# stcodeer/Frequency-wised_All-in-One_Image_Restoration_Model

Measured on AMD Instinct MI355X. Metric: training images/sec @128x128, higher is better.
Workload: dtype bf16; 1 GPU; BASELINE configs[1]: Uformer encoder+decoder (all_3_bands, L=3, freq MSA), denoise sigma=25, 128x128, phase-2 train step (fwd+bwd+Adam, DropPath on); per_gpu_batch=16, global_batch=16, parallelism=dp1, hip_graph=True

## Files before the change

frequency-wised_all-in-one_image_restoration_model_amd/csrc/fw_common.h:

```cpp
#pragma once
#include <hip/hip_runtime.h>
#include <stdint.h>
#include <mutex>

#define FW_DT_F32 0
#define FW_DT_BF16 1

typedef __attribute__((ext_vector_type(4))) float f32x4;
typedef __attribute__((ext_vector_type(8))) __bf16 bf16x8_t;
typedef unsigned short bf16raw;

#define FW_DEV static __device__ __forceinline__
#define FW_SPEC __device__ __forceinline__
#define FW_MEM __device__ __forceinline__

FW_DEV int lane_id() { return threadIdx.x & 63; }

FW_DEV float bf2f(bf16raw b) { return __uint_as_float(((unsigned)b) << 16); }
FW_DEV bf16raw f2bf(float f) {
    __bf16 h = (__bf16)f;
    return __builtin_bit_cast(bf16raw, h);
}
typedef __attribute__((ext_vector_type(2))) float fw_f32x2;
typedef __attribute__((ext_vector_type(2))) __bf16 fw_bf16x2;
// ... 139 lines not shown
}
template <> FW_SPEC void store_acc_T<bf16raw>(char* dst, int ldb, int row0, int col0, const f32x4& acc) {
    const int l = lane_id();
    uint2 v = make_uint2(pack_bf2(acc[0], acc[1]), pack_bf2(acc[2], acc[3]));
    *reinterpret_cast<uint2*>(dst + (col0 + (l & 15)) * ldb + (row0 + ((l >> 4) << 2)) * 2) = v;
}
template <typename T> FW_DEV void store_acc_N(char* dst, int ldb, int row0, int col0, const f32x4& acc) {
    const int l = lane_id();
    char* p = dst + (row0 + ((l >> 4) << 2)) * ldb + (col0 + (l & 15)) * TT<T>::SZ;
#pragma unroll
    for (int r = 0; r < 4; ++r) TT<T>::st(reinterpret_cast<T*>(p + r * ldb), acc[r]);
}

template <typename T, int MT, int NT>
FW_DEV void mma_tiles(f32x4 (&acc)[MT][NT], const char* A, int lda, int a_row0, const char* B, int ldb,
                      int b_row0, int KC) {
    for (int c = 0; c < KC; ++c) {
        uint4 af[MT], bfr[NT];
#pragma unroll
        for (int m = 0; m < MT; ++m) af[m] = frag_kc(A, lda, a_row0 + 16 * m, c);
#pragma unroll
        for (int n = 0; n < NT; ++n) bfr[n] = frag_kc(B, ldb, b_row0 + 16 * n, c);
#pragma unroll
        for (int m = 0; m < MT; ++m)
#pragma unroll
            for (int n = 0; n < NT; ++n) mma_chunk<T>(acc[m][n], af[m], bfr[n]);
    }
}

template <int MT, int NT> FW_DEV void zero_acc(f32x4 (&acc)[MT][NT]) {
#pragma unroll
    for (int m = 0; m < MT; ++m)
#pragma unroll
        for (int n = 0; n < NT; ++n) acc[m][n] = f32x4{0.f, 0.f, 0.f, 0.f};
}

#define FW_MFMA_F32(acc, a, b) acc = __builtin_amdgcn_mfma_f32_16x16x4f32(a, b, acc, 0, 0, 0)

FW_DEV f32x4 frag_g(const float* P, int pitch, int row0, int c) {
    const int l = lane_id();
    return *reinterpret_cast<const f32x4*>(P + (size_t)(row0 + (l & 15)) * pitch + c * 16 + ((l >> 4) << 2));
}

template <bool REAL_IN, bool REAL_OUT, bool PANEL_FIRST> struct DftChunk {
    f32x4 ar[2], ai[2], pc[2], p1[2], p2[2];
    FW_MEM void load_panels(int t, const float* P, int pitch, int p0, int c, bool conj) {
        const size_t plane = (size_t)pitch * pitch;
        pc[t] = frag_g(P, pitch, p0 + 16 * t, c);
        if (!REAL_IN) p1[t] = frag_g(P + (conj ? 2 : 1) * plane, pitch, p0 + 16 * t, c);
        if (!REAL_OUT) p2[t] = frag_g(P + (conj ? 1 : 2) * plane, pitch, p0 + 16 * t, c);
    }
    FW_MEM void load_data(int t, const float* xr, const float* xi, int pitch, int d0, int c) {
        ar[t] = frag_g(xr, pitch, d0 + 16 * t, c);
        if (!REAL_IN) ai[t] = frag_g(xi, pitch, d0 + 16 * t, c);
    }
    FW_MEM void load(const float* xr, const float* xi, int dpitch, int d0, const float* P, int ppitch, int p0, int c, bool conj) {
#pragma unroll
        for (int t = 0; t < 2; ++t) {
            load_data(t, xr, xi, dpitch, d0, c);
            load_panels(t, P, ppitch, p0, c, conj);
        }
    }
    FW_MEM void mac(f32x4 (&accr)[2][2], f32x4 (&acci)[2][2]) const {
#pragma unroll
        for (int s = 0; s < 4; ++s)
#pragma unroll
            for (int mt = 0; mt < 2; ++mt)
#pragma unroll
                for (int nt = 0; nt < 2; ++nt) {
                    const int d = PANEL_FIRST ? nt : mt, p = PANEL_FIRST ? mt : nt;
#define FW_CHUNK_MAC(acc, x, pn) FW_MFMA_F32(acc, PANEL_FIRST ? pn[p][s] : x[d][s], PANEL_FIRST ? x[d][s] : pn[p][s])
                    FW_CHUNK_MAC(accr[mt][nt], ar, pc);
                    if (!REAL_OUT) FW_CHUNK_MAC(acci[mt][nt], ar, p2);
                    if (!REAL_IN) {
                        FW_CHUNK_MAC(accr[mt][nt], ai, p1);
                        if (!REAL_OUT) FW_CHUNK_MAC(acci[mt][nt], ai, pc);
                    }
#undef FW_CHUNK_MAC
                }
    }
    FW_MEM void mac(f32x4 (&acc)[2][2]) const { mac(acc, acc); }
};

#define FW_CHECK_ARG(cond)                                                                   \
    do {                                                                                     \
        if (!(cond)) return -__LINE__;                                                       \
    } while (0)
#define FW_LAUNCH_RET()                                                                      \
    do {                                                                                     \
        hipError_t e__ = hipGetLastError();                                                  \
        return e__ == hipSuccess ? 0 : (int)e__;                                             \
    } while (0)

#define FW_SET_LDS_ONCE(kern, bytes)                                                         \
    do {                                                                                     \
        static std::once_flag once__;                                                        \
        std::call_once(once__, [&] {                                                         \
            (void)hipFuncSetAttribute(reinterpret_cast<const void*>(kern), hipFuncAttributeMaxDynamicSharedMemorySize, (int)(bytes)); \
        });                                                                                  \
    } while (0)

static inline int fw_cdiv(long a, long b) { return (int)((a + b - 1) / b); }
```

frequency-wised_all-in-one_image_restoration_model_amd/csrc/fw_elem.hip:

```cpp
#include "fw_common.h"
#include <stdlib.h>

namespace {

constexpr int TPB = 256;
FW_DEV long gtid() { return (long)blockIdx.x * TPB + threadIdx.x; }
FW_DEV long gstride() { return (long)gridDim.x * TPB; }
static inline int grid_for(long n, int cap = 8192) { long g = (n + TPB - 1) / TPB; return (int)(g < 1 ? 1 : (g > cap ? cap : g)); }

template <typename T> FW_DEV void ldvec(const T* p, float* f) {
    unpack16<T>(*reinterpret_cast<const uint4*>(p), f);
}
template <typename T> FW_DEV void stvec(T* p, const float* f) { *reinterpret_cast<uint4*>(p) = pack16<T>(f); }
template <typename T> FW_DEV void ldvec4(const T* p, float* f);
template <> FW_SPEC void ldvec4<float>(const float* p, float* f) { unpack16<float>(*reinterpret_cast<const uint4*>(p), f); }
template <> FW_SPEC void ldvec4<bf16raw>(const bf16raw* p, float* f) {
    const uint2 v = *reinterpret_cast<const uint2*>(p);
    f[0] = __uint_as_float(v.x << 16); f[1] = __uint_as_float(v.x & 0xffff0000u);
    f[2] = __uint_as_float(v.y << 16); f[3] = __uint_as_float(v.y & 0xffff0000u);
}
template <typename T> FW_DEV void stvec4(T* p, const float* f);
template <> FW_SPEC void stvec4<float>(float* p, const float* f) { *reinterpret_cast<uint4*>(p) = pack16<float>(f); }
template <> FW_SPEC void stvec4<bf16raw>(bf16raw* p, const float* f) {
    *reinterpret_cast<uint2*>(p) = make_uint2(pack_bf2(f[0], f[1]), pack_bf2(f[2], f[3]));
// ... 712 lines not shown
        else *reinterpret_cast<uint2*>(d) = make_uint2(pack_bf2(v[0], v[1]), pack_bf2(v[2], v[3]));
    }
}
template <typename T>
__global__ void col2im4_kernel(const T* __restrict__ dcol, float* __restrict__ dx, long lddx, const float* __restrict__ dres, long ldr,
                               int B, int H, int W, int C) {
    const int Ho = H / 2, Wo = W / 2, c4n = C >> 2;
    const long total = (long)B * H * W * c4n;
    for (long i = gtid(); i < total; i += gstride()) {
        const int c = (int)(i % c4n) * 4; const long tok = i / c4n;
        const int x = (int)(tok % W); const int y = (int)((tok / W) % H); const long b = tok / ((long)W * H);
        f32x4 acc = f32x4{0.f, 0.f, 0.f, 0.f};
        if (dres) acc = *reinterpret_cast<const f32x4*>(dres + tok * ldr + c);
        for (int ky = (y + 1) & 1; ky < 4; ky += 2) {
            const int oy = (y + 1 - ky) / 2;
            if (y + 1 - ky < 0 || oy >= Ho) continue;
            for (int kx = (x + 1) & 1; kx < 4; kx += 2) {
                const int ox = (x + 1 - kx) / 2;
                if (x + 1 - kx < 0 || ox >= Wo) continue;
                const T* s = dcol + (((b * Ho + oy) * Wo + ox) * 16 + ky * 4 + kx) * (long)C + c;
                for (int e = 0; e < 4; ++e) acc[e] += TT<T>::ld(s + e);
            }
        }
        *reinterpret_cast<f32x4*>(dx + tok * lddx + c) = acc;
    }
}

template <typename T>
__global__ __launch_bounds__(1024) void im2col4_run_kernel(const float* __restrict__ x, long ldx, T* __restrict__ col, int B, int H, int W, int C,
                                                           int ipb) {
    const int Ho = H / 2, Wo = W / 2, c4n = C >> 2, Q = 4 * c4n;
    const int il = threadIdx.x / Q, q = threadIdx.x - il * Q;
    if (il >= ipb) return;
    const int kx = q / c4n, c = (q - kx * c4n) * 4;
    const unsigned ntok = (unsigned)B * Ho * Wo;
    for (unsigned t = blockIdx.x * ipb + il; t < ntok; t += gridDim.x * ipb) {
        const unsigned ox = t % Wo, t2 = t / Wo, oy = t2 % Ho, b = t2 / Ho;
        const int ix = 2 * (int)ox - 1 + kx, iy0 = 2 * (int)oy - 1;
        const bool okx = ix >= 0 && ix < W;
        const float* px = x + (((long)b * H) * W + min(max(ix, 0), W - 1)) * ldx + c;
        f32x4 v[4];
#pragma unroll
        for (int ky = 0; ky < 4; ++ky) v[ky] = *reinterpret_cast<const f32x4*>(px + (long)min(max(iy0 + ky, 0), H - 1) * W * ldx);
        T* d = col + ((long)t * 16 + kx) * C + c;
#pragma unroll
        for (int ky = 0; ky < 4; ++ky) {
            const bool ok = okx && iy0 + ky >= 0 && iy0 + ky < H;
            const f32x4 u = ok ? v[ky] : f32x4{0.f, 0.f, 0.f, 0.f};
            if (sizeof(T) == 4) *reinterpret_cast<f32x4*>(d + (long)ky * 4 * C) = u;
            else *reinterpret_cast<uint2*>(d + (long)ky * 4 * C) = make_uint2(pack_bf2(u[0], u[1]), pack_bf2(u[2], u[3]));
        }
    }
}
template <typename T>
__global__ __launch_bounds__(1024) void col2im4_run_kernel(const T* __restrict__ dcol, float* __restrict__ dx, long lddx, const float* __restrict__ dres,
                                                           long ldr, int B, int H, int W, int C, int ipb) {
    const int Ho = H / 2, Wo = W / 2, c4n = C >> 2;
    const int il = threadIdx.x / c4n, c = (threadIdx.x - il * c4n) * 4;
    if (il >= ipb) return;
    const unsigned ntok = (unsigned)B * H * W;
    for (unsigned tok = blockIdx.x * ipb + il; tok < ntok; tok += gridDim.x * ipb) {
        const unsigned xx = tok % W, t2 = tok / W, yy = t2 % H, b = t2 / H;
        const int x = (int)xx, y = (int)yy;
        const int ky0 = (y + 1) & 1, kx0 = (x + 1) & 1;
        float f[4][4];
        bool ok[4];
#pragma unroll
        for (int i = 0; i < 2; ++i)
#pragma unroll
            for (int j = 0; j < 2; ++j) {
                const int ky = ky0 + 2 * i, kx = kx0 + 2 * j;
                const int ny = y + 1 - ky, nx = x + 1 - kx;
                ok[i * 2 + j] = ny >= 0 && ny < 2 * Ho && nx >= 0 && nx < 2 * Wo;
                const int oy = min(max(ny, 0) >> 1, Ho - 1), ox = min(max(nx, 0) >> 1, Wo - 1);
                ldvec4<T>(dcol + ((((long)b * Ho + oy) * Wo + ox) * 16 + ky * 4 + kx) * (long)C + c, f[i * 2 + j]);
            }
        f32x4 acc = f32x4{0.f, 0.f, 0.f, 0.f};
        if (dres) acc = *reinterpret_cast<const f32x4*>(dres + (long)tok * ldr + c);
#pragma unroll
        for (int k = 0; k < 4; ++k)
#pragma unroll
            for (int e = 0; e < 4; ++e) acc[e] = ok[k] ? acc[e] + f[k][e] : acc[e];
        *reinterpret_cast<f32x4*>(dx + (long)tok * lddx + c) = acc;
    }
}

template <typename T>
__global__ void pixel_shuffle_kernel(const T* __restrict__ g, const float* __restrict__ bias, float* __restrict__ out, long ldo,
                                     int B, int H, int W, int Cout) {
    const int c4n = Cout >> 2;
    const long total = (long)B * H * W * 4 * c4n;
    for (long i = gtid(); i < total; i += gstride()) {
        const int c = (int)(i % c4n) * 4; long t = i / c4n;
        const int q = (int)(t % 4); t /= 4;
        const int x = (int)(t % W); const int y = (int)((t / W) % H); const long b = t / ((long)W * H);
        const T* s = g + t * 4L * Cout + q * Cout + c;
        float* d = out + ((b * 2 * H + 2 * y + (q >> 1)) * 2 * W + 2 * x + (q & 1)) * ldo + c;
        f32x4 v;
        for (int e = 0; e < 4; ++e) v[e] = TT<T>::ld(s + e) + bias[c + e];
        *reinterpret_cast<f32x4*>(d) = v;
    }
}
template <typename T>
__global__ void pixel_unshuffle_kernel(const float* __restrict__ dout, long ldo, T* __restrict__ dg, int B, int H, int W, int Cout) {
    const int c4n = Cout >> 2;
    const long total = (long)B * H * W * 4 * c4n;
    for (long i = gtid(); i < total; i += gstride()) {
        const int c = (int)(i % c4n) * 4; long t = i / c4n;
        const int q = (int)(t % 4); t /= 4;
        const int x = (int)(t % W); const int y = (int)((t / W) % H); const long b = t / ((long)W * H);
        const float* s = dout + ((b * 2 * H + 2 * y + (q >> 1)) * 2 * W + 2 * x + (q & 1)) * ldo + c;
        T* d = dg + t * 4L * Cout + q * Cout + c;
        for (int e = 0; e < 4; ++e) TT<T>::st(d + e, s[e]);
    }
}
__global__ void colsum_kernel(const float* __restrict__ x, long ldx, float* __restrict__ out, long rows, int cols, int rows_per_block) {
    const long r0 = (long)blockIdx.x * rows_per_block;
    for (int c = threadIdx.x; c < cols; c += TPB) {
        float s = 0.f;
        for (long r = r0; r < rows && r < r0 + rows_per_block; ++r) s += x[r * ldx + c];
        atomicAdd(out + c, s);
    }
}
__global__ __launch_bounds__(256) void colsum4_kernel(const float* __restrict__ x, long ldx, float* __restrict__ out, long rows, int cols, int rows_per_block) {
    __shared__ f32x4 red[TPB];
    const int nv = cols >> 2, rl = TPB / nv;
    const int v = threadIdx.x % nv, lane = threadIdx.x / nv;
    const long r0 = (long)blockIdx.x * rows_per_block;
    const long r1 = r0 + rows_per_block < rows ? r0 + rows_per_block : rows;
    f32x4 s = f32x4{0.f, 0.f, 0.f, 0.f};
    if (lane < rl) {
#pragma unroll 4
        for (long r = r0 + lane; r < r1; r += rl) s += *reinterpret_cast<const f32x4*>(x + r * ldx + 4 * v);
    }
    red[threadIdx.x] = s;
    __syncthreads();
    if (threadIdx.x < nv) {
        f32x4 t = red[threadIdx.x];
        for (int j = 1; j < rl; ++j) t += red[j * nv + threadIdx.x];
#pragma unroll
        for (int e = 0; e < 4; ++e) atomicAdd(out + 4 * threadIdx.x + e, t[e]);
    }
}
template <typename T>
__global__ void colsum_t_kernel(const T* __restrict__ x, long ldx, float* __restrict__ out, long rows, int cols, int rows_per_block) {
    const long r0 = (long)blockIdx.x * rows_per_block;
    for (int c = threadIdx.x; c < cols; c += TPB) {
        float s = 0.f;
        for (long r = r0; r < rows && r < r0 + rows_per_block; ++r) s += TT<T>::ld(x + r * ldx + c);
        atomicAdd(out + c, s);
    }
}

constexpr int EC_TY = 8, EC_TX = 32, EC_PH = EC_TY + 2, EC_PW = EC_TX + 2, EC_PLANE = EC_PH * EC_PW, EC_PN = 3 * EC_PLANE, EC_PIX = EC_TY * EC_TX;
constexpr int EC_PREG = (EC_PN + 255) / 256;
struct EcTiles {
    int tx, ty; long n;
    __device__ EcTiles(int B, int H, int W) : tx((W + EC_TX - 1) / EC_TX), ty((H + EC_TY - 1) / EC_TY) { n = (long)B * tx * ty; }
    __device__ void at(long t, long& b, int& y0, int& x0) const { x0 = (int)(t % tx) * EC_TX; y0 = (int)((t / tx) % ty) * EC_TY; b = t / ((long)tx * ty); }
};
FW_DEV void ec_patch_load(float (&r)[EC_PREG], const float* __restrict__ src, const EcTiles& T, long t, int H, int W) {
    long b; int y0, x0;
    T.at(t, b, y0, x0);
#pragma unroll
    for (int k = 0; k < EC_PREG; ++k) {
        int i = threadIdx.x + k * 256; i = i < EC_PN ? i : EC_PN - 1;
// ... 505 lines not shown
    FW_CHECK_ARG(dh2 && h1 && w && dh1 && dw && dbias && C % e == 0 && ld1 % e == 0 && ldg % e == 0 && ldo % e == 0 && W % SX == 0);
    FW_CHECK_ARG(ldg == ld1);
    FW_CHECK_ARG(B > 0 && H > 0 && W > 0 && C > 0 && ld1 >= C && ldo >= C);
    const long n = (long)B * H * (W / SX) * (C / 4);
    const int nvg = (C / 4 + WG_VL - 1) / WG_VL;
    const long nst = (long)B * H * (W / SX);
    constexpr int NSTRIP_MAX = 16;
    constexpr long wg_min_blocks = 384;
    int NSTRIP = NSTRIP_MAX;
    while (NSTRIP > 2 && ((nst + (long)NSTRIP * WG_SL - 1) / ((long)NSTRIP * WG_SL)) * nvg < wg_min_blocks) NSTRIP >>= 1;
    const long nsg = (nst + (long)NSTRIP * WG_SL - 1) / ((long)NSTRIP * WG_SL);
    const dim3 gridw((unsigned)(nsg * nvg));
    const bool tiled = dw_tiled(B, H, W, C);
    if (tiled && !g1 && (long)H * W * ldg < (1L << 31)) {
        constexpr long want = 1024;
        const long ncol = (long)((C + DT_CB - 1) / DT_CB) * ((W + DT_TX - 1) / DT_TX), nrow = (long)B * (H / DT_TY);
        long NT = ncol * nrow / want;
        NT = NT < 1 ? 1 : (NT > 32 ? 32 : NT);
        long nb = ncol * ((nrow + NT - 1) / NT);
        nb = (nb + 7) / 8 * 8;
        const size_t esz = dtype == FW_DT_BF16 ? 2 : 4;
        const size_t lds = (size_t)(DT_TY + 2) * ((DT_TX + 2) * DT_CB * esz + 128) + (9 * DT_CB + 40 * 256) * sizeof(float);
        if (dtype == FW_DT_BF16) {
            FW_SET_LDS_ONCE((dwconv_bwd_fused_kernel<bf16raw>), lds);
            hipLaunchKernelGGL((dwconv_bwd_fused_kernel<bf16raw>), dim3((unsigned)nb), dim3(256), lds, ST, (const bf16raw*)dh2, ldg, (const bf16raw*)h1, w,
                               (bf16raw*)dh1, ldo, dw, dbias, B, H, W, C, (int)NT);
        } else {
            FW_SET_LDS_ONCE((dwconv_bwd_fused_kernel<float>), lds);
            hipLaunchKernelGGL((dwconv_bwd_fused_kernel<float>), dim3((unsigned)nb), dim3(256), lds, ST, (const float*)dh2, ldg, (const float*)h1, w,
                               (float*)dh1, ldo, dw, dbias, B, H, W, C, (int)NT);
        }
        FW_LAUNCH_RET();
    }
    if (tiled) {
        const int rc = dtype == FW_DT_BF16
            ? dwconv_tile_launch<bf16raw, 1>((const bf16raw*)dh2, ldg, w, (const float*)nullptr, (const bf16raw*)h1, (bf16raw*)dh1, (bf16raw*)nullptr, ldo, B, H, W, C, ST)
            : dwconv_tile_launch<float, 1>((const float*)dh2, ldg, w, (const float*)nullptr, (const float*)h1, (float*)dh1, (float*)nullptr, ldo, B, H, W, C, ST);
        if (rc) return rc;
    }
    if (dtype == FW_DT_BF16) {
        if (!tiled) hipLaunchKernelGGL((dwconv_strip_kernel<bf16raw, 1>), dim3((grid_for(n) + 7) / 8 * 8), dim3(TPB), 0, ST, (const bf16raw*)dh2, ldg, w, (const float*)nullptr,
                           (const bf16raw*)h1, (bf16raw*)dh1, (bf16raw*)nullptr, ldo, B, H, W, C);
        if (g1) hipLaunchKernelGGL((dwconv_wgrad_kernel<bf16raw, false>), gridw, dim3(256), 0, ST, (const bf16raw*)dh2, ldg, (const bf16raw*)g1, ld1, dw, dbias, B, H, W, C, NSTRIP);
        else hipLaunchKernelGGL((dwconv_wgrad_kernel<bf16raw, true>), gridw, dim3(256), 0, ST, (const bf16raw*)dh2, ldg, (const bf16raw*)h1, ld1, dw, dbias, B, H, W, C, NSTRIP);
    } else {
        if (!tiled) hipLaunchKernelGGL((dwconv_strip_kernel<float, 1>), dim3((grid_for(n) + 7) / 8 * 8), dim3(TPB), 0, ST, (const float*)dh2, ldg, w, (const float*)nullptr,
                           (const float*)h1, (float*)dh1, (float*)nullptr, ldo, B, H, W, C);
        if (g1) hipLaunchKernelGGL((dwconv_wgrad_kernel<float, false>), gridw, dim3(256), 0, ST, (const float*)dh2, ldg, (const float*)g1, ld1, dw, dbias, B, H, W, C, NSTRIP);
        else hipLaunchKernelGGL((dwconv_wgrad_kernel<float, true>), gridw, dim3(256), 0, ST, (const float*)dh2, ldg, (const float*)h1, ld1, dw, dbias, B, H, W, C, NSTRIP);
    }
    FW_LAUNCH_RET();
}
extern "C" int fw_im2col4(int dtype, const float* x, long ldx, void* col, int B, int H, int W, int C, void* stream) {
    FW_CHECK_ARG(x && col && C % 4 == 0 && ldx % 4 == 0 && H % 2 == 0 && W % 2 == 0);
    const long n = (long)B * (H / 2) * (W / 2) * 16 * (C / 4);
    const long ntok = (long)B * (H / 2) * (W / 2);
    if (C >= 4 && C <= 1024 && ntok > 0 && ntok < (1L << 31) - (1L << 24) && ((uintptr_t)x & 15) == 0 &&
        ((uintptr_t)col & (dtype == FW_DT_BF16 ? 7 : 15)) == 0) {
        const int ipb = C >= 256 ? 1 : 256 / C;
        const dim3 g((unsigned)run_grid(ntok, ipb)), b((unsigned)((ipb * C + 63) / 64 * 64));
        if (dtype == FW_DT_BF16) hipLaunchKernelGGL((im2col4_run_kernel<bf16raw>), g, b, 0, ST, x, ldx, (bf16raw*)col, B, H, W, C, ipb);
        else hipLaunchKernelGGL((im2col4_run_kernel<float>), g, b, 0, ST, x, ldx, (float*)col, B, H, W, C, ipb);
        FW_LAUNCH_RET();
    }
    if (dtype == FW_DT_BF16) LAUNCH((im2col4_kernel<bf16raw>), n, x, ldx, (bf16raw*)col, B, H, W, C);
    LAUNCH((im2col4_kernel<float>), n, x, ldx, (float*)col, B, H, W, C);
}
extern "C" int fw_col2im4(int dtype, const void* dcol, float* dx, long lddx, const float* dres, long ldr, int B, int H, int W, int C,
                          void* stream) {
    FW_CHECK_ARG(dcol && dx && C % 4 == 0 && lddx % 4 == 0 && H % 2 == 0 && W % 2 == 0 && (!dres || ldr % 4 == 0));
    const long n = (long)B * H * W * (C / 4);
    const long ntok = (long)B * H * W;
    if (C >= 4 && C <= 4096 && ntok > 0 && ntok < (1L << 31) - (1L << 24) && (((uintptr_t)dx | (uintptr_t)dres) & 15) == 0 &&
        ((uintptr_t)dcol & (dtype == FW_DT_BF16 ? 7 : 15)) == 0) {
        const int c4n = C / 4, ipb = c4n >= 256 ? 1 : 256 / c4n;
        const dim3 g((unsigned)run_grid(ntok, ipb)), b((unsigned)((ipb * c4n + 63) / 64 * 64));
        if (dtype == FW_DT_BF16) hipLaunchKernelGGL((col2im4_run_kernel<bf16raw>), g, b, 0, ST, (const bf16raw*)dcol, dx, lddx, dres, ldr, B, H, W, C, ipb);
        else hipLaunchKernelGGL((col2im4_run_kernel<float>), g, b, 0, ST, (const float*)dcol, dx, lddx, dres, ldr, B, H, W, C, ipb);
        FW_LAUNCH_RET();
    }
    if (dtype == FW_DT_BF16) LAUNCH((col2im4_kernel<bf16raw>), n, (const bf16raw*)dcol, dx, lddx, dres, ldr, B, H, W, C);
    LAUNCH((col2im4_kernel<float>), n, (const float*)dcol, dx, lddx, dres, ldr, B, H, W, C);
}
extern "C" int fw_pixel_shuffle(int dtype, const void* g, const float* bias, float* out, long ldo, int B, int H, int W, int Cout,
                                void* stream) {
    FW_CHECK_ARG(g && bias && out && Cout % 4 == 0 && ldo % 4 == 0);
    const long n = (long)B * H * W * Cout;
    if (dtype == FW_DT_BF16) LAUNCH((pixel_shuffle_kernel<bf16raw>), n, (const bf16raw*)g, bias, out, ldo, B, H, W, Cout);
    LAUNCH((pixel_shuffle_kernel<float>), n, (const float*)g, bias, out, ldo, B, H, W, Cout);
}
extern "C" int fw_pixel_unshuffle(int dtype, const float* dout, long ldo, void* dg, int B, int H, int W, int Cout, void* stream) {
    FW_CHECK_ARG(dout && dg && Cout % 4 == 0 && ldo % 4 == 0);
    const long n = (long)B * H * W * Cout;
    if (dtype == FW_DT_BF16) LAUNCH((pixel_unshuffle_kernel<bf16raw>), n, dout, ldo, (bf16raw*)dg, B, H, W, Cout);
    LAUNCH((pixel_unshuffle_kernel<float>), n, dout, ldo, (float*)dg, B, H, W, Cout);
}
extern "C" int fw_colsum(int x_dtype, const void* x, long ldx, float* out, long rows, int cols, void* stream) {
    FW_CHECK_ARG(x && out && rows > 0 && cols > 0);
    int rpb = (int)((rows + 1023) / 1024);
    if (rpb < 32) rpb = 32;
    int grid = (int)((rows + rpb - 1) / rpb);
    if (x_dtype != 1 && cols % 4 == 0 && cols <= 512 && ldx % 4 == 0 && ((uintptr_t)x & 15) == 0 && ((uintptr_t)out & 3) == 0) {
        rpb = (int)((rows + 255) / 256);
        if (rpb < 32) rpb = 32;
        grid = (int)((rows + rpb - 1) / rpb);
        hipLaunchKernelGGL(colsum4_kernel, dim3(grid), dim3(TPB), 0, ST, (const float*)x, ldx, out, rows, cols, rpb);
        FW_LAUNCH_RET();
    }
    if (x_dtype == 1) hipLaunchKernelGGL((colsum_t_kernel<bf16raw>), dim3(grid), dim3(TPB), 0, ST, (const bf16raw*)x, ldx, out, rows, cols, rpb);
    else hipLaunchKernelGGL(colsum_kernel, dim3(grid), dim3(TPB), 0, ST, (const float*)x, ldx, out, rows, cols, rpb);
    FW_LAUNCH_RET();
}
#ifndef FW_EC_WGRAD_CAP
#define FW_EC_WGRAD_CAP 512
#endif
static inline int ec_grid(int B, int H, int W, int cap) {
    const long n = (long)B * ((H + EC_TY - 1) / EC_TY) * ((W + EC_TX - 1) / EC_TX);
    return (int)(n < cap ? n : cap);
}
static inline bool ec_al16(const void* p) { return ((uintptr_t)p & 15) == 0; }
constexpr int OP_PROD_BYTES = ((EC_PLANE + 15) / 16) * 16 * OP_PS * 4;
constexpr int OP_MAX_C = 896;
extern "C" int fw_inproj_fwd(const float* img, const float* w, const float* bias, float* out, long ldo, int B, int H, int W, int C,
                             float slope, void* stream) {
    FW_CHECK_ARG(img && w && bias && out && C % 4 == 0 && ldo % 4 == 0 && C > 0 && C <= 1024 && B > 0 && H > 0 && W > 0);
    FW_CHECK_ARG(ec_al16(out) && ec_al16(bias));
    hipLaunchKernelGGL(edge_conv3_rows_kernel<0>, dim3(ec_grid(B, H, W, 768)), dim3(TPB), 0, ST, img, w, bias, out, ldo, B, H, W, C, slope);
    FW_LAUNCH_RET();
}
extern "C" int fw_inproj_bwd(const float* img, const float* out, long ldo, const float* dy, long ldy, float* dw, float* db, int B,
                             int H, int W, int C, float slope, void* stream) {
    FW_CHECK_ARG(img && out && dy && dw && db && C > 0 && B > 0 && H > 0 && W > 0);
    const dim3 grid(ec_grid(B, H, W, FW_EC_WGRAD_CAP));
    const bool v4 = C % 4 == 0 && ldo % 4 == 0 && ldy % 4 == 0 && ec_al16(out) && ec_al16(dy);
    const int slice = v4 ? 1024 : 256;
    for (int c0 = 0; c0 < C; c0 += slice) {
        const int cs = C - c0 < slice ? C - c0 : slice;
        if (v4) hipLaunchKernelGGL((edge_conv3_wgrad_kernel<4, 0>), grid, dim3(TPB), 0, ST, img, dy + c0, ldy, out + c0, ldo, dw + (long)c0 * 27, db + c0, B, H, W, cs, slope);
        else hipLaunchKernelGGL((edge_conv3_wgrad_kernel<1, 0>), grid, dim3(TPB), 0, ST, img, dy + c0, ldy, out + c0, ldo, dw + (long)c0 * 27, db + c0, B, H, W, cs, slope);
    }
    FW_LAUNCH_RET();
}
extern "C" int fw_outproj_fwd(const float* fea, long ldf, const float* w, const float* bias, const float* img, float* out, int B,
                              int H, int W, int C, void* stream) {
    FW_CHECK_ARG(fea && w && bias && out && C % 4 == 0 && ldf % 4 == 0 && C > 0 && C <= OP_MAX_C && B > 0 && H > 0 && W > 0 && ec_al16(fea));
    const size_t lds = (size_t)((C + 15) / 16) * 2048 + OP_PROD_BYTES;
    FW_SET_LDS_ONCE(outproj_fwd_mfma_kernel, (OP_MAX_C / 16) * 2048 + OP_PROD_BYTES);
    hipLaunchKernelGGL(outproj_fwd_mfma_kernel, dim3(ec_grid(B, H, W, 512)), dim3(TPB), lds, ST, fea, ldf, w, bias, img, out, B, H, W, C);
    FW_LAUNCH_RET();
}
extern "C" int fw_outproj_bwd(const float* dout, const float* fea, long ldf, const float* w, float* dfea, long lddf, float* dw,
                              float* db, int B, int H, int W, int C, void* stream) {
    FW_CHECK_ARG(dout && fea && w && dfea && dw && db && C % 4 == 0 && ldf % 4 == 0 && lddf % 4 == 0 && C > 0 && C <= 1024 && B > 0 && H > 0 && W > 0);
    FW_CHECK_ARG(ec_al16(fea) && ec_al16(dfea));
    hipLaunchKernelGGL(edge_conv3_rows_kernel<1>, dim3(ec_grid(B, H, W, 768)), dim3(TPB), 0, ST, dout, w, (const float*)nullptr, dfea, lddf, B, H, W, C, 0.f);
    hipLaunchKernelGGL((edge_conv3_wgrad_kernel<4, 1>), dim3(ec_grid(B, H, W, FW_EC_WGRAD_CAP)), dim3(TPB), 0, ST, dout, fea, ldf, (const float*)nullptr, 0L, dw, db,
                       B, H, W, C, 0.f);
    FW_LAUNCH_RET();
}
extern "C" int fw_l1_loss(const float* a, const float* b, float* da, long n, float gscale, float* loss, void* stream) {
    FW_CHECK_ARG(a && b && loss && n > 0);
    const int vec = (((uintptr_t)a | (uintptr_t)b | (uintptr_t)da) & 15) == 0;
    hipLaunchKernelGGL(l1_loss_kernel, dim3(grid_for(vec ? (n + 3) / 4 : n, 512)), dim3(TPB), 0, ST, a, b, da, n, gscale, loss, vec);
    FW_LAUNCH_RET();
}
extern "C" int fw_ce0_loss(const float* logits, float* dlogits, int R, int N, float gscale, float* loss, void* stream) {
// ... 62 lines not shown
```

frequency-wised_all-in-one_image_restoration_model_amd/csrc/fw_gemm.hip:

```cpp
#include "fw_common.h"
#include <stdio.h>
#include <string.h>
#include <stdlib.h>

namespace {
static thread_local char g_last_kernel[96] = "";
template <typename T> constexpr const char* tname() { return sizeof(T) == 2 ? "bf16" : "float"; }
#define FW_B(x) ((x) ? "true" : "false")
#define FW_KNAME(...) snprintf(g_last_kernel, sizeof g_last_kernel, __VA_ARGS__)

struct GemmArgs {
    const char* X; const char* W; char* C;
    long ldx, ldw, ldc;
    int M, N, K;
    int x_op, w_op;
    const float* bias;
    int act; float slope;
    const char* aux; long ldaux;
    const float* rowscale; int rows_per_scale;
    const float* residual; long ldr;
    int out_f32;
    int accumulate;
    int splitk; int kper;
    char* C2; long ldc2;
    float* xsum;
    long c_zstride, xsum_zstride;
    float alpha;
    int staged;
    int dbg;
};

constexpr int LDS_ROW = 128;
FW_DEV int swz(int row) { return ((row ^ (row >> 3)) & 7) << 4; }
constexpr int BM = 128;

FW_DEV unsigned xcd_contiguous(unsigned lin, unsigned total) {
    const unsigned xcd = lin & 7, q = total >> 3, r = total & 7;
    return (xcd < r ? xcd * (q + 1) : r * (q + 1) + (xcd - r) * q) + (lin >> 3);
}

template <typename T> FW_DEV uint4 apply_gelu16(const uint4& v) {
    float f[TT<T>::E16];
    unpack16<T>(v, f);
#pragma unroll
    for (int i = 0; i < TT<T>::E16; ++i) f[i] = gelu_t<T>(f[i]);
    return pack16<T>(f);
}

template <typename T>
FW_DEV void epi_fetch(const GemmArgs& a, uint4& ext, int mc, int nc, int z) {
    if (a.act == 2) {
        const T* ap = reinterpret_cast<const T*>(a.aux) + (long)mc * a.ldaux + nc;
        if (sizeof(T) == 4) ext = *reinterpret_cast<const uint4*>(ap);
        else { const uint2 t = *reinterpret_cast<const uint2*>(ap); ext.x = t.x; ext.y = t.y; }
    } else if (a.residual && z == 0) {
        ext = *reinterpret_cast<const uint4*>(a.residual + (long)mc * a.ldr + nc);
    }
}
FW_DEV f32x4 epi_bias(const GemmArgs& a, int nc, int z) {
    return (a.bias && z == 0) ? *reinterpret_cast<const f32x4*>(a.bias + nc) : f32x4{0.f, 0.f, 0.f, 0.f};
}
template <typename T>
FW_DEV void epi_apply(const GemmArgs& a, const f32x4& bias, const uint4& ext, const f32x4& acc, int m, int n0, float rs, int z) {
    float v[4];
#pragma unroll
    for (int r = 0; r < 4; ++r) v[r] = acc[r] * a.alpha + bias[r];
    if (a.act == 1) {
#pragma unroll
        for (int r = 0; r < 4; ++r) v[r] = lrelu_f(v[r], a.slope);
    } else if (a.act == 2) {
        float x[4];
        if (sizeof(T) == 4) { x[0] = __uint_as_float(ext.x); x[1] = __uint_as_float(ext.y); x[2] = __uint_as_float(ext.z); x[3] = __uint_as_float(ext.w); }
        else { x[0] = __uint_as_float(ext.x << 16); x[1] = __uint_as_float(ext.x & 0xffff0000u);
               x[2] = __uint_as_float(ext.y << 16); x[3] = __uint_as_float(ext.y & 0xffff0000u); }
#pragma unroll
        for (int r = 0; r < 4; ++r) v[r] *= gelu_grad_t<T>(x[r]);
    } else if (a.act == 3) {
#pragma unroll
        for (int r = 0; r < 4; ++r) v[r] = gelu_t<T>(v[r]);
    }
    if (a.rowscale) {
#pragma unroll
        for (int r = 0; r < 4; ++r) v[r] *= rs;
    }
    if (a.residual && z == 0) {
        uint4 rr = ext;
        if (a.act == 2) rr = *reinterpret_cast<const uint4*>(a.residual + (long)m * a.ldr + n0);
        v[0] += __uint_as_float(rr.x); v[1] += __uint_as_float(rr.y); v[2] += __uint_as_float(rr.z); v[3] += __uint_as_float(rr.w);
    }
    if (a.C2) {
        T* c2 = reinterpret_cast<T*>(a.C2) + (long)m * a.ldc2 + n0;
        const float g0 = gelu_t<T>(v[0]), g1 = gelu_t<T>(v[1]), g2 = gelu_t<T>(v[2]), g3 = gelu_t<T>(v[3]);
        if (sizeof(T) == 4) *reinterpret_cast<f32x4*>(c2) = f32x4{g0, g1, g2, g3};
        else *reinterpret_cast<uint2*>(c2) = make_uint2(pack_bf2(g0, g1), pack_bf2(g2, g3));
    }
    if (a.out_f32) {
        float* cp = reinterpret_cast<float*>(a.C) + (long)z * a.c_zstride + (long)m * a.ldc + n0;
        if (a.accumulate && a.c_zstride == 0) {
            if (a.accumulate == 1 && a.splitk == 1) {
                const f32x4 old = *reinterpret_cast<const f32x4*>(cp);
                *reinterpret_cast<f32x4*>(cp) = f32x4{old[0] + v[0], old[1] + v[1], old[2] + v[2], old[3] + v[3]};
            } else {
#pragma unroll
                for (int r = 0; r < 4; ++r) atomicAdd(cp + r, v[r]);
            }
        } else {
            *reinterpret_cast<f32x4*>(cp) = f32x4{v[0], v[1], v[2], v[3]};
        }
    } else {
        T* cp = reinterpret_cast<T*>(a.C) + (long)m * a.ldc + n0;
        if (sizeof(T) == 4) *reinterpret_cast<f32x4*>(cp) = f32x4{v[0], v[1], v[2], v[3]};
        else *reinterpret_cast<uint2*>(cp) = make_uint2(pack_bf2(v[0], v[1]), pack_bf2(v[2], v[3]));
// ... 406 lines not shown
            }
        };
        auto apply = [&](const uint4 (&ext)[4], int mt) {
            const int m = m_blk + wm0 + mt * 16 + (l & 15);
            const int mc = m < a.M ? m : a.M - 1;
            const float rs = a.rowscale ? a.rowscale[mc / a.rows_per_scale] : 1.0f;
#pragma unroll
            for (int nt = 0; nt < 4; ++nt) {
                const int n0 = n_blk + wn0 + nt * 16 + ((l >> 4) << 2);
                if (m < a.M && n0 < a.N) epi_apply<T>(a, bias4[nt], ext[nt], acc[nt][mt], m, n0, rs, bz);
            }
        };
        uint4 ea[4], eb[4];
        fetch(ea, 0);
#pragma unroll
        for (int mt = 0; mt < WM; mt += 2) {
            if (mt + 1 < WM) fetch(eb, mt + 1);
            apply(ea, mt);
            if (mt + 1 < WM) {
                if (mt + 2 < WM) fetch(ea, mt + 2);
                apply(eb, mt + 1);
            }
        }
    }
}
static inline bool plain_epilogue(const GemmArgs& a) {
    return a.act == 0 && !a.rowscale && !a.residual && !a.C2 && a.alpha == 1.0f && !(a.accumulate && a.c_zstride == 0);
}

template <int N> FW_DEV void wait_vmcnt() { asm volatile("s_waitcnt vmcnt(%0)" ::"n"(N) : "memory"); }
FW_DEV void glds16_asm(const char* gsrc, char* lds_dst) {
    unsigned keep;
    const unsigned dst = __builtin_amdgcn_readfirstlane((unsigned)(uintptr_t)(lds_void_t*)lds_dst);
    asm volatile("s_mov_b32 %0, m0\n\ts_mov_b32 m0, %2\n\ts_nop 0\n\tglobal_load_lds_dwordx4 %1, off\n\ts_mov_b32 m0, %0"
                 : "=&s"(keep) : "v"(gsrc), "s"(dst) : "memory");
}

template <int KT> struct GldsKm {
    static constexpr int NI = KT / 16;
    const char* src[NI];
    long kstride;
    int loff[NI];
    FW_MEM void init(const char* base, long ld, int col0, int cols_total, int k0) {
        const int lane = threadIdx.x & 63, wave = threadIdx.x >> 6;
        kstride = ld * 2;
#pragma unroll
        for (int it = 0; it < NI; ++it) {
            const int R0 = wave * (KT / 4) + it * 4;
            const int r = R0 + (lane >> 4), p = lane & 15;
            int col = col0 + ((p ^ swz256(r)) << 3);
            if (col >= cols_total) col = 0;
            src[it] = base + ((long)(k0 + r) * ld + col) * 2;
            loff[it] = R0 * 256;
        }
    }
    FW_MEM void issue(int step, char* tile) const {
        const long off = (long)step * KT * kstride;
#pragma unroll
        for (int it = 0; it < NI; ++it) glds16_asm(src[it] + off, tile + loff[it]);
    }
};
template <typename T, int ROWS> struct GldsKc {
    static constexpr int NI = ROWS / 32;
    const char* src[NI];
    int loff[NI];
    FW_MEM void init(const char* base, long ld, int row0, int rows_total, int kbyte0) {
        const int lane = threadIdx.x & 63, wave = threadIdx.x >> 6;
#pragma unroll
        for (int it = 0; it < NI; ++it) {
            const int R0 = (wave * NI + it) * 8;
            const int r = R0 + (lane >> 3), p = lane & 7;
            int gr = row0 + r;
            if (gr >= rows_total) gr = rows_total - 1;
            src[it] = base + (long)gr * ld * TT<T>::SZ + kbyte0 + ((p ^ (swz(r) >> 4)) << 4);
            loff[it] = R0 * LDS_ROW;
        }
    }
    FW_MEM void issue(int step, char* tile) const {
#pragma unroll
        for (int it = 0; it < NI; ++it) glds16_asm(src[it] + (long)step * 128, tile + loff[it]);
    }
};

constexpr int ROW64 = 64;
FW_DEV int swz64(int r) { return (r >> 2) & 3; }
template <typename T, int ROWS> struct GldsKc64 {
    static constexpr int NI = ROWS / 64;
    const char* src[NI];
    int loff[NI];
    FW_MEM void init(const char* base, long ld, int row0, int rows_total, int kbyte0) {
        const int lane = threadIdx.x & 63, wave = threadIdx.x >> 6;
#pragma unroll
        for (int it = 0; it < NI; ++it) {
            const int R0 = (wave * NI + it) * 16;
            const int r = R0 + (lane >> 2), p = lane & 3;
            int gr = row0 + r;
            if (gr >= rows_total) gr = rows_total - 1;
            src[it] = base + (long)gr * ld * TT<T>::SZ + kbyte0 + ((p ^ swz64(r)) << 4);
            loff[it] = R0 * ROW64;
        }
    }
    FW_MEM void issue(int step, char* tile) const {
#pragma unroll
        for (int it = 0; it < NI; ++it) glds16_asm(src[it] + (long)step * ROW64, tile + loff[it]);
    }
};
FW_DEV uint4 frag_sw64(const char* tile, int row0) {
    const int l = lane_id();
    const int row = row0 + (l & 15);
    return *reinterpret_cast<const uint4*>(tile + row * ROW64 + (((l >> 4) ^ swz64(row)) << 4));
}

constexpr int EPI_LD = 136;
template <int WM>
FW_DEV void tile_epilogue_staged(const GemmArgs& a, const f32x4 (&acc)[4][WM], int m_blk, int n_blk, int wm0, int wn0, char* stage, int mode) {
    const int l = lane_id();
    char* mine = stage + (threadIdx.x >> 6) * (16 * WM * EPI_LD);
    f32x4 bias4[4];
#pragma unroll
    for (int nt = 0; nt < 4; ++nt) {
        const int n0 = n_blk + wn0 + nt * 16 + ((l >> 4) << 2);
        bias4[nt] = epi_bias(a, n0 < a.N ? n0 : 0, 0);
    }
    const int rsub = l >> 3, cb = (l & 7) * 16;
    const int ncol = n_blk + wn0 + (l & 7) * 8;
    const bool col_ok = ncol < a.N;
    auto rows_out = [&](char* C, long ldc) {
#pragma unroll
        for (int it = 0; it < 2 * WM; ++it) {
            const int r = it * 8 + rsub, m = m_blk + wm0 + r;
            const uint4 v = *reinterpret_cast<const uint4*>(mine + r * EPI_LD + cb);
            if (m < a.M && col_ok) *reinterpret_cast<uint4*>(C + ((long)m * ldc + ncol) * 2) = v;
        }
    };
    if (mode == 2) {
#pragma unroll
        for (int it = 0; it < 2 * WM; ++it) {
            const int r = it * 8 + rsub, m = m_blk + wm0 + r;
            const long mc = m < a.M ? m : a.M - 1;
            const uint4 v = *reinterpret_cast<const uint4*>(a.aux + (mc * a.ldaux + (col_ok ? ncol : 0)) * 2);
            *reinterpret_cast<uint4*>(mine + r * EPI_LD + cb) = v;
        }
        __builtin_amdgcn_fence(__ATOMIC_RELEASE, "wavefront");
        asm volatile("s_waitcnt vmcnt(0) lgkmcnt(0)" ::: "memory");
        __builtin_amdgcn_fence(__ATOMIC_ACQUIRE, "wavefront");
    }
#pragma unroll
    for (int pass = 0; pass < 2; ++pass) {
        if (pass == 1 && mode != 1) break;
#pragma unroll
        for (int mt = 0; mt < WM; ++mt) {
            char* rowp = mine + (mt * 16 + (l & 15)) * EPI_LD + ((l >> 4) << 3);
#pragma unroll
            for (int nt = 0; nt < 4; ++nt) {
                f32x4 v = acc[nt][mt] + bias4[nt];
                if (mode == 2) {
                    const uint2 e = *reinterpret_cast<const uint2*>(rowp + nt * 32);
                    v[0] *= gelu_grad_poly(__uint_as_float(e.x << 16)); v[1] *= gelu_grad_poly(__uint_as_float(e.x & 0xffff0000u));
                    v[2] *= gelu_grad_poly(__uint_as_float(e.y << 16)); v[3] *= gelu_grad_poly(__uint_as_float(e.y & 0xffff0000u));
                } else if (pass == 1) {
                    v[0] = gelu_poly(v[0]); v[1] = gelu_poly(v[1]); v[2] = gelu_poly(v[2]); v[3] = gelu_poly(v[3]);
                }
                *reinterpret_cast<uint2*>(rowp + nt * 32) = make_uint2(pack_bf2(v[0], v[1]), pack_bf2(v[2], v[3]));
            }
        }
        __builtin_amdgcn_fence(__ATOMIC_RELEASE, "wavefront");
        asm volatile("s_waitcnt lgkmcnt(0)" ::: "memory");
        __builtin_amdgcn_fence(__ATOMIC_ACQUIRE, "wavefront");
        if (pass == 0) rows_out(a.C, a.ldc); else rows_out(a.C2, a.ldc2);
        if (pass == 0 && mode == 1) {
            __builtin_amdgcn_fence(__ATOMIC_RELEASE, "wavefront");
            asm volatile("s_waitcnt lgkmcnt(0)" ::: "memory");
            __builtin_amdgcn_fence(__ATOMIC_ACQUIRE, "wavefront");
        }
    }
}
static inline int staged_mode(const GemmArgs& a) {
    if (a.out_f32 || a.alpha != 1.0f || a.rowscale || a.residual || a.accumulate || a.c_zstride || a.splitk != 1 || a.N % 8 || a.ldc % 8) return -1;
    if (((uintptr_t)a.C & 15)) return -1;
    if (a.act == 0 && !a.C2) return 0;
    if (a.act == 0 && a.C2) return (a.ldc2 % 8 || ((uintptr_t)a.C2 & 15)) ? -1 : 1;
    if (a.act == 2 && !a.C2) return (a.ldaux % 8 || ((uintptr_t)a.aux & 15)) ? -1 : 2;
    return -1;
}

template <bool XT, int KT, int NS, bool PLAIN>
FW_DEV void tr_ring_tile(const GemmArgs& a, int bx, int by, int bz, char* smem) {
    using T = bf16raw;
    static_assert(NS == 2 || NS == 3, "ring depth");
    constexpr int WM = 4;
    constexpr bool X64 = !XT && KT == 32;
    constexpr int XB = XT ? KT * 256 : 128 * (X64 ? ROW64 : LDS_ROW), WB = KT * 256, STAGE = XB + WB;
    constexpr int LPS = (XT ? KT / 16 : (X64 ? 2 : 4)) + KT / 16;
    auto xs = [&](int i) -> char* { return smem + i * STAGE; };
    auto ws = [&](int i) -> char* { return smem + i * STAGE + XB; };
    const int wave = threadIdx.x >> 6;
    const int m_blk = bx * 128, n_blk = by * 128;
    const int wm0 = (wave & 1) * 64, wn0 = (wave >> 1) * 64;
    const int k_begin = bz * a.kper;
    const int k_end = min(a.K, k_begin + a.kper);
    const int nsteps = (k_end - k_begin) / KT;

    f32x4 acc[4][WM], xsacc[WM];
    zero_acc(acc);
#pragma unroll
    for (int m = 0; m < WM; ++m) xsacc[m] = f32x4{0.f, 0.f, 0.f, 0.f};
    const bool do_xsum = XT && a.xsum != nullptr && by == 0 && wn0 == 0;
    const uint4 ones = make_uint4(0x3F803F80u, 0x3F803F80u, 0x3F803F80u, 0x3F803F80u);

    GldsKm<KT> gw;
    gw.init(a.W, a.ldw, n_blk, a.N, k_begin);
    GldsKm<XT ? KT : 16> gxm;
    GldsKc<T, BM> gxc;
    GldsKc64<T, BM> gxc64;
    if constexpr (XT) gxm.init(a.X, a.ldx, m_blk, a.M, k_begin);
    else if constexpr (X64) gxc64.init(a.X, a.ldx, m_blk, a.M, k_begin * 2);
    else gxc.init(a.X, a.ldx, m_blk, a.M, k_begin * 2);
    auto issue = [&](int step, int buf) {
        if constexpr (XT) gxm.issue(step, xs(buf));
        else if constexpr (X64) gxc64.issue(step, xs(buf));
        else gxc.issue(step, xs(buf));
        gw.issue(step, ws(buf));
    };
#pragma unroll
    for (int p = 0; p < NS - 1; ++p)
        if (p < nsteps) issue(p, p);
    int buf = 0;
    for (int s = 0; s < nsteps; ++s) {
        const int younger = min(NS - 2, nsteps - 1 - s);
        if (younger >= NS - 2) wait_vmcnt<(NS - 2) * LPS>();
        else wait_vmcnt<0>();
        __builtin_amdgcn_s_barrier();
        asm volatile("" ::: "memory");
        if (s + NS - 1 < nsteps) issue(s + NS - 1, buf == 0 ? NS - 1 : buf - 1);
#pragma unroll
        for (int c = 0; c < KT / 32; ++c) {
            uint4 af[4], bfr[WM];
#pragma unroll
            for (int m = 0; m < 4; ++m) af[m] = frag_tr256(ws(buf), wn0 + 16 * m, c);
#pragma unroll
            for (int n = 0; n < WM; ++n) bfr[n] = XT ? frag_tr256(xs(buf), wm0 + 16 * n, c) : (X64 ? frag_sw64(xs(buf), wm0 + 16 * n) : frag_sw(xs(buf), wm0 + 16 * n, c));
#pragma unroll
            for (int m = 0; m < 4; ++m)
#pragma unroll
                for (int n = 0; n < WM; ++n) mma_chunk<T>(acc[m][n], af[m], bfr[n]);
            if (do_xsum) {
#pragma unroll
                for (int n = 0; n < WM; ++n) mma_chunk<T>(xsacc[n], ones, bfr[n]);
            }
        }
        buf = buf + 1 == NS ? 0 : buf + 1;
    }
    const int l = lane_id();
    if (do_xsum && (l >> 4) == 0) {
#pragma unroll
        for (int n = 0; n < WM; ++n) {
            const int m = m_blk + wm0 + n * 16 + l;
            if (m < a.M) {
                if (a.xsum_zstride > 0) a.xsum[(long)bz * a.xsum_zstride + m] = xsacc[n][0];
                else atomicAdd(a.xsum + m, xsacc[n][0]);
            }
        }
    }
    if (a.staged >= 0 && (size_t)NS * STAGE >= (size_t)4 * 16 * WM * EPI_LD) {
        __syncthreads();
        tile_epilogue_staged<WM>(a, acc, m_blk, n_blk, wm0, wn0, smem, a.staged);
        return;
    }
    tile_epilogue<T, WM, PLAIN>(a, acc, m_blk, n_blk, wm0, wn0, bz);
}

template <bool XT, int KT, int NS, bool PLAIN>
__global__ __launch_bounds__(256, KT == 32 ? 3 : 2) void gemm_tr_ring_kernel(GemmArgs a) {
    extern __shared__ __attribute__((aligned(16))) char smem[];
    int bx = blockIdx.x, by = blockIdx.y, bz = blockIdx.z;
    {
        const unsigned total = gridDim.x * gridDim.y * gridDim.z;
        if (gridDim.z > 1) {
            const unsigned lin = blockIdx.x + gridDim.x * (blockIdx.y + gridDim.y * blockIdx.z);
            const unsigned w = xcd_contiguous(lin, total);
            bx = (int)(w % gridDim.x);
            by = (int)((w / gridDim.x) % gridDim.y);
            bz = (int)(w / (gridDim.x * gridDim.y));
        } else if (gridDim.z == 1 && gridDim.y > 1) {
            const unsigned lin = blockIdx.x + gridDim.x * blockIdx.y;
            const unsigned w = xcd_contiguous(lin, total);
            const unsigned per_band = 8 * gridDim.y;
            const unsigned band = w / per_band, first = band * 8;
            const unsigned gsz = min(gridDim.x - first, 8u);
            bx = (int)(first + (w % per_band) % gsz);
            by = (int)((w % per_band) / gsz);
        }
    }
    tr_ring_tile<XT, KT, NS, PLAIN>(a, bx, by, bz, smem);
}

__global__ __launch_bounds__(256, 3) void gemm_wgrad_group_kernel(const GemmArgs* __restrict__ probs, const int4* __restrict__ items) {
    extern __shared__ __attribute__((aligned(16))) char smem[];
    const int4 it = items[blockIdx.x];
    if (it.x < 0) return;
    const GemmArgs a = probs[it.x];
    if (a.c_zstride > 0) tr_ring_tile<true, 32, 3, true>(a, it.y, it.z, it.w, smem);
    else tr_ring_tile<true, 32, 3, false>(a, it.y, it.z, it.w, smem);
}

template <bool PLAIN>
FW_DEV void tr_big_tile(const GemmArgs& a, int bx, int by, int bz, char* smem) {
    using T = bf16raw;
    constexpr int KT = 32, NS = 3, WM = 8, IMG = KT * 256, STAGE = 4 * IMG, LPS = 4;
    const int lane = threadIdx.x & 63, wave = threadIdx.x >> 6;
    const int m_blk = bx * 256, n_blk = by * 256;
    const int wm0 = (wave & 1) * 128, wn0 = (wave >> 1) * 64;
    const int k_begin = bz * a.kper;
    const int k_end = min(a.K, k_begin + a.kper);
    const int nsteps = (k_end - k_begin) / KT;
    const char* src[4]; int off[4];
    {
        const bool isw = wave >= 4;
        const int half = (wave >> 1) & 1, rg = wave & 1;
        const char* base = isw ? a.W : a.X;
        const long ld = isw ? a.ldw : a.ldx;
        const int col0 = (isw ? n_blk : m_blk) + half * 128, cols = isw ? a.N : a.M;
#pragma unroll
        for (int it = 0; it < 4; ++it) {
            const int R0 = rg * 16 + it * 4, r = R0 + (lane >> 4), p = lane & 15;
            int col = col0 + ((p ^ swz256(r)) << 3);
            if (col >= cols) col = 0;
            src[it] = base + ((long)(k_begin + r) * ld + col) * 2;
            off[it] = (isw ? 2 * IMG : 0) + half * IMG + R0 * 256;
        }
    }
    const long kstride = (wave >= 4 ? a.ldw : a.ldx) * 2;
    auto issue = [&](int step, int buf) {
        char* st = smem + buf * STAGE;
#pragma unroll
        for (int it = 0; it < 4; ++it) glds16_asm(src[it] + (long)step * KT * kstride, st + off[it]);
    };
    f32x4 acc[4][WM];
    zero_acc(acc);
    float xs[WM];
#pragma unroll
    for (int m = 0; m < WM; ++m) xs[m] = 0.f;
    const bool do_xsum = a.xsum != nullptr && by == 0 && wn0 == 0;
    typedef __attribute__((ext_vector_type(2))) __bf16 bf2_t;
    const bf2_t ones2 = __builtin_bit_cast(bf2_t, 0x3F803F80u);
#pragma unroll
    for (int p = 0; p < NS - 1; ++p)
        if (p < nsteps) issue(p, p);
    int buf = 0;
    for (int s = 0; s < nsteps; ++s) {
        const int younger = min(NS - 2, nsteps - 1 - s);
        if (younger >= NS - 2) wait_vmcnt<(NS - 2) * LPS>();
        else wait_vmcnt<0>();
        __builtin_amdgcn_s_barrier();
        asm volatile("" ::: "memory");
        if (s + NS - 1 < nsteps) issue(s + NS - 1, buf == 0 ? NS - 1 : buf - 1);
        const char* st = smem + buf * STAGE;
        uint4 af[4], bfr[WM];
#pragma unroll
        for (int m = 0; m < 4; ++m) af[m] = frag_tr256(st + 2 * IMG + (wn0 >> 7) * IMG, (wn0 & 127) + 16 * m, 0);
#pragma unroll
        for (int n = 0; n < WM; ++n) bfr[n] = frag_tr256(st + (wm0 >> 7) * IMG, 16 * n, 0);
#pragma unroll
        for (int m = 0; m < 4; ++m)
#pragma unroll
            for (int n = 0; n < WM; ++n) mma_chunk<T>(acc[m][n], af[m], bfr[n]);
        if (do_xsum) {
#pragma unroll
            for (int n = 0; n < WM; ++n) {
                xs[n] = __builtin_amdgcn_fdot2_f32_bf16(__builtin_bit_cast(bf2_t, bfr[n].x), ones2, xs[n], false);
                xs[n] = __builtin_amdgcn_fdot2_f32_bf16(__builtin_bit_cast(bf2_t, bfr[n].y), ones2, xs[n], false);
                xs[n] = __builtin_amdgcn_fdot2_f32_bf16(__builtin_bit_cast(bf2_t, bfr[n].z), ones2, xs[n], false);
                xs[n] = __builtin_amdgcn_fdot2_f32_bf16(__builtin_bit_cast(bf2_t, bfr[n].w), ones2, xs[n], false);
            }
        }
        buf = buf + 1 == NS ? 0 : buf + 1;
    }
    const int l = lane_id();
    if (do_xsum) {
#pragma unroll
        for (int n = 0; n < WM; ++n) {
            float v = xs[n];
            v += __shfl_xor(v, 16, 64); v += __shfl_xor(v, 32, 64);
            const int m = m_blk + wm0 + n * 16 + l;
            if ((l >> 4) == 0 && m < a.M) {
                if (a.xsum_zstride > 0) a.xsum[(long)bz * a.xsum_zstride + m] = v;
                else atomicAdd(a.xsum + m, v);
            }
        }
    }
    tile_epilogue<T, WM, PLAIN>(a, acc, m_blk, n_blk, wm0, wn0, bz);
}
__global__ __launch_bounds__(512) void gemm_wgrad_group_big_kernel(const GemmArgs* __restrict__ probs, const int4* __restrict__ items) {
    extern __shared__ __attribute__((aligned(16))) char smem[];
    const int4 it = items[blockIdx.x];
    if (it.x < 0) return;
    const GemmArgs a = probs[it.x];
    if (a.c_zstride > 0) tr_big_tile<true>(a, it.y, it.z, it.w, smem);
    else tr_big_tile<false>(a, it.y, it.z, it.w, smem);
}

template <bool XT, int KT, int NS, bool PLAIN>
int launch_tr_ring_p(const GemmArgs& a, hipStream_t st) {
    const size_t lds = (size_t)NS * ((XT ? KT * 256 : 128 * ((KT == 32) ? ROW64 : LDS_ROW)) + KT * 256);
    FW_SET_LDS_ONCE((gemm_tr_ring_kernel<XT, KT, NS, PLAIN>), lds);
    FW_KNAME("gemm_tr_ring_kernel<%s,%d,%d,%s>", FW_B(XT), KT, NS, FW_B(PLAIN));
    hipLaunchKernelGGL((gemm_tr_ring_kernel<XT, KT, NS, PLAIN>), dim3(fw_cdiv(a.M, 128), fw_cdiv(a.N, 128), a.splitk), dim3(256), lds, st, a);
    FW_LAUNCH_RET();
}
template <bool XT, int KT, int NS>
int launch_tr_ring(const GemmArgs& a, hipStream_t st) {
    return plain_epilogue(a) ? launch_tr_ring_p<XT, KT, NS, true>(a, st) : launch_tr_ring_p<XT, KT, NS, false>(a, st);
}

template <typename T, int BN, int NS, bool PLAIN>
__global__ __launch_bounds__(256) void gemm_ring_kernel(GemmArgs a) {
    constexpr int KT = 128 / TT<T>::SZ;
    constexpr int WM = (BN == 128) ? 4 : 2;
    constexpr int XBYTES = BM * LDS_ROW, WBYTES = BN * LDS_ROW, STAGE = XBYTES + WBYTES;
    constexpr int LPS = BM / 32 + BN / 32;
    extern __shared__ __attribute__((aligned(16))) char smem[];
    auto xs = [&](int i) -> char* { return smem + i * STAGE; };
    auto ws = [&](int i) -> char* { return smem + i * STAGE + XBYTES; };
    const int wave = threadIdx.x >> 6;
    int bx = blockIdx.x, by = blockIdx.y, bz = blockIdx.z;
    {
        const unsigned total = gridDim.x * gridDim.y * gridDim.z;
        if (gridDim.z > 1) {
            const unsigned lin = blockIdx.x + gridDim.x * (blockIdx.y + gridDim.y * blockIdx.z);
            const unsigned w = xcd_contiguous(lin, total);
            bx = (int)(w % gridDim.x);
            by = (int)((w / gridDim.x) % gridDim.y);
            bz = (int)(w / (gridDim.x * gridDim.y));
        } else if (gridDim.z == 1 && gridDim.y > 1) {
            const unsigned lin = blockIdx.x + gridDim.x * blockIdx.y;
            const unsigned w = xcd_contiguous(lin, total);
            const unsigned per_band = 8 * gridDim.y;
            const unsigned band = w / per_band, first = band * 8;
            const unsigned gsz = min(gridDim.x - first, 8u);
            bx = (int)(first + (w % per_band) % gsz);
            by = (int)((w % per_band) / gsz);
        }
    }
    const int m_blk = bx * BM, n_blk = by * BN;
    const int wm0 = (BN == 128) ? (wave & 1) * 64 : wave * 32;
    const int wn0 = (BN == 128) ? (wave >> 1) * 64 : 0;
    const int k_begin = bz * a.kper;
    const int k_end = min(a.K, k_begin + a.kper);
    const int nsteps = (k_end - k_begin) / KT;

    f32x4 acc[4][WM];
    zero_acc(acc);
    GldsKc<T, BM> gx;
    GldsKc<T, BN> gw;
    gx.init(a.X, a.ldx, m_blk, a.M, k_begin * TT<T>::SZ);
    gw.init(a.W, a.ldw, n_blk, a.N, k_begin * TT<T>::SZ);
    auto issue = [&](int step, int buf) {
        gx.issue(step, xs(buf));
        gw.issue(step, ws(buf));
    };
#pragma unroll
    for (int p = 0; p < NS - 1; ++p)
        if (p < nsteps) issue(p, p);
    int buf = 0;
    for (int s = 0; s < nsteps; ++s) {
        const int younger = min(NS - 2, nsteps - 1 - s);
        if (younger >= NS - 2) wait_vmcnt<(NS - 2) * LPS>();
        else wait_vmcnt<0>();
        __builtin_amdgcn_s_barrier();
        asm volatile("" ::: "memory");
        if (s + NS - 1 < nsteps) issue(s + NS - 1, buf == 0 ? NS - 1 : buf - 1);
#pragma unroll
        for (int c = 0; c < 2; ++c) {
            uint4 af[4], bfr[WM];
#pragma unroll
            for (int m = 0; m < 4; ++m) af[m] = frag_sw(ws(buf), wn0 + 16 * m, c);
#pragma unroll
            for (int n = 0; n < WM; ++n) bfr[n] = frag_sw(xs(buf), wm0 + 16 * n, c);
#pragma unroll
            for (int m = 0; m < 4; ++m)
#pragma unroll
                for (int n = 0; n < WM; ++n) mma_chunk<T>(acc[m][n], af[m], bfr[n]);
        }
        buf = buf + 1 == NS ? 0 : buf + 1;
    }
    if constexpr (sizeof(T) == 2) {
        if (a.staged >= 0 && (size_t)NS * STAGE >= (size_t)4 * 16 * WM * EPI_LD) {
            __syncthreads();
            tile_epilogue_staged<WM>(a, acc, m_blk, n_blk, wm0, wn0, smem, a.staged);
            return;
        }
    }
    tile_epilogue<T, WM, PLAIN>(a, acc, m_blk, n_blk, wm0, wn0, bz);
}

template <typename T, int BN, int NS, bool PLAIN>
int launch_ring_p(const GemmArgs& a, hipStream_t st) {
    const size_t lds = (size_t)NS * (BM + BN) * LDS_ROW;
    FW_SET_LDS_ONCE((gemm_ring_kernel<T, BN, NS, PLAIN>), lds);
    dim3 grid(fw_cdiv(a.M, BM), fw_cdiv(a.N, BN), a.splitk);
    FW_KNAME("gemm_ring_kernel<%s,%d,%d,%s>", tname<T>(), BN, NS, FW_B(PLAIN));
    hipLaunchKernelGGL((gemm_ring_kernel<T, BN, NS, PLAIN>), grid, dim3(256), lds, st, a);
    FW_LAUNCH_RET();
}
template <typename T, int BN, int NS>
int launch_ring(const GemmArgs& a, hipStream_t st) {
    return plain_epilogue(a) ? launch_ring_p<T, BN, NS, true>(a, st) : launch_ring_p<T, BN, NS, false>(a, st);
}

template <typename T, int BN, int NS, bool PLAIN>
__global__ __launch_bounds__(256) void gemm_ring64_kernel(GemmArgs a) {
    constexpr int KT = ROW64 / TT<T>::SZ;
    constexpr int WM = (BN == 128) ? 4 : 2;
    constexpr int XBYTES = BM * ROW64, WBYTES = BN * ROW64, STAGE = XBYTES + WBYTES;
    constexpr int LPS = BM / 64 + BN / 64;
    static_assert(NS >= 3, "ring depth");
    extern __shared__ __attribute__((aligned(16))) char smem[];
    auto xs = [&](int i) -> char* { return smem + i * STAGE; };
    auto ws = [&](int i) -> char* { return smem + i * STAGE + XBYTES; };
    const int wave = threadIdx.x >> 6;
    int bx = blockIdx.x, by = blockIdx.y, bz = blockIdx.z;
    {
        const unsigned total = gridDim.x * gridDim.y * gridDim.z;
        if (gridDim.z > 1) {
            const unsigned lin = blockIdx.x + gridDim.x * (blockIdx.y + gridDim.y * blockIdx.z);
            const unsigned w = xcd_contiguous(lin, total);
            bx = (int)(w % gridDim.x);
            by = (int)((w / gridDim.x) % gridDim.y);
            bz = (int)(w / (gridDim.x * gridDim.y));
        } else if (gridDim.z == 1 && gridDim.y > 1) {
            const unsigned lin = blockIdx.x + gridDim.x * blockIdx.y;
            const unsigned w = xcd_contiguous(lin, total);
            const unsigned per_band = 8 * gridDim.y;
            const unsigned band = w / per_band, first = band * 8;
            const unsigned gsz = min(gridDim.x - first, 8u);
            bx = (int)(first + (w % per_band) % gsz);
            by = (int)((w % per_band) / gsz);
        }
    }
    const int m_blk = bx * BM, n_blk = by * BN;
    const int wm0 = (BN == 128) ? (wave & 1) * 64 : wave * 32;
    const int wn0 = (BN == 128) ? (wave >> 1) * 64 : 0;
    const int k_begin = bz * a.kper;
    const int k_end = min(a.K, k_begin + a.kper);
    const int nsteps = (k_end - k_begin) / KT;

    f32x4 acc[4][WM];
    zero_acc(acc);
    GldsKc64<T, BM> gx;
    GldsKc64<T, BN> gw;
    gx.init(a.X, a.ldx, m_blk, a.M, k_begin * TT<T>::SZ);
    gw.init(a.W, a.ldw, n_blk, a.N, k_begin * TT<T>::SZ);
    auto issue = [&](int step, int buf) {
        gx.issue(step, xs(buf));
        gw.issue(step, ws(buf));
    };
#pragma unroll
    for (int p = 0; p < NS - 1; ++p)
        if (p < nsteps) issue(p, p);
    int buf = 0;
    for (int s = 0; s < nsteps; ++s) {
        const int younger = min(NS - 2, nsteps - 1 - s);
        if (younger >= NS - 2) wait_vmcnt<(NS - 2) * LPS>();
        else if (younger == NS - 3) wait_vmcnt<(NS - 3) * LPS>();
        else wait_vmcnt<0>();
        __builtin_amdgcn_s_barrier();
        asm volatile("" ::: "memory");
        if (s + NS - 1 < nsteps) issue(s + NS - 1, buf == 0 ? NS - 1 : buf - 1);
        uint4 af[4], bfr[WM];
#pragma unroll
        for (int m = 0; m < 4; ++m) af[m] = frag_sw64(ws(buf), wn0 + 16 * m);
#pragma unroll
        for (int n = 0; n < WM; ++n) bfr[n] = frag_sw64(xs(buf), wm0 + 16 * n);
#pragma unroll
        for (int m = 0; m < 4; ++m)
#pragma unroll
            for (int n = 0; n < WM; ++n) mma_chunk<T>(acc[m][n], af[m], bfr[n]);
        buf = buf + 1 == NS ? 0 : buf + 1;
    }
    if constexpr (sizeof(T) == 2) {
        if (a.staged >= 0 && (size_t)NS * STAGE >= (size_t)4 * 16 * WM * EPI_LD) {
            __syncthreads();
            tile_epilogue_staged<WM>(a, acc, m_blk, n_blk, wm0, wn0, smem, a.staged);
            return;
        }
    }
    tile_epilogue<T, WM, PLAIN>(a, acc, m_blk, n_blk, wm0, wn0, bz);
}

template <typename T, int BN, int NS, bool PLAIN>
int launch_ring64_p(const GemmArgs& a, hipStream_t st) {
    const size_t lds = (size_t)NS * (BM + BN) * ROW64;
    FW_SET_LDS_ONCE((gemm_ring64_kernel<T, BN, NS, PLAIN>), lds);
    dim3 grid(fw_cdiv(a.M, BM), fw_cdiv(a.N, BN), a.splitk);
    FW_KNAME("gemm_ring64_kernel<%s,%d,%d,%s>", tname<T>(), BN, NS, FW_B(PLAIN));
    hipLaunchKernelGGL((gemm_ring64_kernel<T, BN, NS, PLAIN>), grid, dim3(256), lds, st, a);
    FW_LAUNCH_RET();
}
template <typename T, int BN, int NS>
int launch_ring64(const GemmArgs& a, hipStream_t st) {
    return plain_epilogue(a) ? launch_ring64_p<T, BN, NS, true>(a, st) : launch_ring64_p<T, BN, NS, false>(a, st);
}

template <bool WT, bool PLAIN>
__global__ __launch_bounds__(512) void gemm_big_kernel(GemmArgs a) {
    using T = bf16raw;
    constexpr int KT = 64, NS = 2, WM = 8, BIG = 256;
    constexpr int XB = BIG * LDS_ROW, WB = WT ? 2 * KT * 256 : XB, STAGE = XB + WB;
    constexpr int NIX = 4, NIW = 4, LPS = NIX + NIW;
    extern __shared__ __attribute__((aligned(16))) char smem[];
    auto xs = [&](int i) -> char* { return smem + i * STAGE; };
    auto ws = [&](int i) -> char* { return smem + i * STAGE + XB; };
    const int lane = threadIdx.x & 63, wave = threadIdx.x >> 6;
    int bx = blockIdx.x, by = blockIdx.y;
    if (gridDim.y > 1) {
        const unsigned total = gridDim.x * gridDim.y;
        const unsigned lin = blockIdx.x + gridDim.x * blockIdx.y;
        const unsigned w = xcd_contiguous(lin, total);
        const unsigned per_band = 8 * gridDim.y;
        const unsigned band = w / per_band, first = band * 8;
        const unsigned gsz = min(gridDim.x - first, 8u);
        bx = (int)(first + (w % per_band) % gsz);
        by = (int)((w % per_band) / gsz);
    }
    const int m_blk = bx * BIG, n_blk = by * BIG;
    const int wm0 = (wave & 1) * 128, wn0 = (wave >> 1) * 64;
    const int nsteps = a.K / KT;

    const char* xsrc[NIX]; int xoff[NIX];
    const char* wsrc[NIW]; int woff[NIW];
    long wkstride = 0;
#pragma unroll
    for (int it = 0; it < NIX; ++it) {
        const int R0 = (wave * NIX + it) * 8, r = R0 + (lane >> 3), p = lane & 7;
        int gr = m_blk + r; if (gr >= a.M) gr = a.M - 1;
        xsrc[it] = a.X + (long)gr * a.ldx * 2 + ((p ^ (swz(r) >> 4)) << 4);
        xoff[it] = R0 * LDS_ROW;
    }
    if constexpr (!WT) {
#pragma unroll
        for (int it = 0; it < NIW; ++it) {
            const int R0 = (wave * NIW + it) * 8, r = R0 + (lane >> 3), p = lane & 7;
            int gr = n_blk + r; if (gr >= a.N) gr = a.N - 1;
            wsrc[it] = a.W + (long)gr * a.ldw * 2 + ((p ^ (swz(r) >> 4)) << 4);
            woff[it] = R0 * LDS_ROW;
        }
    } else {
        const int half = wave >> 2, wq = wave & 3;
        wkstride = a.ldw * 2;
#pragma unroll
        for (int it = 0; it < NIW; ++it) {
            const int R0 = wq * (KT / 4) + it * 4, r = R0 + (lane >> 4), p = lane & 15;
            int col = n_blk + half * 128 + ((p ^ swz256(r)) << 3);
            if (col >= a.N) col = 0;
            wsrc[it] = a.W + ((long)r * a.ldw + col) * 2;
            woff[it] = half * KT * 256 + R0 * 256;
        }
    }
    auto issue = [&](int step, int buf) {
        char* xt = xs(buf); char* wt = ws(buf);
#pragma unroll
        for (int it = 0; it < NIX; ++it) glds16_asm(xsrc[it] + (long)step * KT * 2, xt + xoff[it]);
#pragma unroll
        for (int it = 0; it < NIW; ++it) glds16_asm(wsrc[it] + (WT ? (long)step * KT * wkstride : (long)step * KT * 2), wt + woff[it]);
    };
    f32x4 acc[4][WM];
    zero_acc(acc);
    const bool noload = a.dbg & 2;
#pragma unroll
    for (int p = 0; p < NS - 1; ++p)
        if (p < nsteps && !noload) issue(p, p);
    int buf = 0;
    for (int s = 0; s < nsteps; ++s) {
        const int younger = min(NS - 2, nsteps - 1 - s);
        if (younger >= NS - 2) wait_vmcnt<(NS - 2) * LPS>();
        else wait_vmcnt<0>();
        __builtin_amdgcn_s_barrier();
        asm volatile("" ::: "memory");
        if (s + NS - 1 < nsteps && !noload) issue(s + NS - 1, buf == 0 ? NS - 1 : buf - 1);
        const char* xt = xs(buf); const char* wt = ws(buf);
#pragma unroll
        for (int c = 0; c < KT / 32; ++c) {
            uint4 af[4], bfr[WM];
#pragma unroll
            for (int m = 0; m < 4; ++m) {
                if constexpr (WT) af[m] = frag_tr256(wt + (wn0 >> 7) * KT * 256, (wn0 & 127) + 16 * m, c);
                else af[m] = frag_sw(wt, wn0 + 16 * m, c);
            }
#pragma unroll
            for (int n = 0; n < WM; ++n) bfr[n] = frag_sw(xt, wm0 + 16 * n, c);
#pragma unroll
            for (int m = 0; m < 4; ++m)
#pragma unroll
                for (int n = 0; n < WM; ++n) mma_chunk<T>(acc[m][n], af[m], bfr[n]);
        }
        buf = buf + 1 == NS ? 0 : buf + 1;
    }
    if ((a.dbg & 1) && acc[0][0][0] != 12345.678f) return;
    if (a.staged >= 0) {
        __syncthreads();
        tile_epilogue_staged<WM>(a, acc, m_blk, n_blk, wm0, wn0, smem, a.staged);
        return;
    }
    tile_epilogue<T, WM, PLAIN>(a, acc, m_blk, n_blk, wm0, wn0, 0);
}

template <bool WT, bool PLAIN>
__global__ __launch_bounds__(256, 2) void gemm_wide_kernel(GemmArgs a) {
    using T = bf16raw;
    constexpr int KT = 32, NS = 3, WM = 8, TM = 128, TN = 256;
    constexpr int XB = TM * ROW64, WB = WT ? 2 * KT * 256 : TN * ROW64, STAGE = XB + WB;
    constexpr int NIX = 2, NIW = 4, LPS = NIX + NIW;
    extern __shared__ __attribute__((aligned(16))) char smem[];
    auto xs = [&](int i) -> char* { return smem + i * STAGE; };
    auto ws = [&](int i) -> char* { return smem + i * STAGE + XB; };
    const int lane = threadIdx.x & 63, wave = threadIdx.x >> 6;
    int bx = blockIdx.x, by = blockIdx.y;
    if (gridDim.y > 1) {
        const unsigned total = gridDim.x * gridDim.y;
        const unsigned lin = blockIdx.x + gridDim.x * blockIdx.y;
        const unsigned w = xcd_contiguous(lin, total);
        const unsigned per_band = 8 * gridDim.y;
        const unsigned band = w / per_band, first = band * 8;
        const unsigned gsz = min(gridDim.x - first, 8u);
        bx = (int)(first + (w % per_band) % gsz);
        by = (int)((w % per_band) / gsz);
    }
    const int m_blk = bx * TM, n_blk = by * TN;
    const int wm0 = 0, wn0 = wave * 64;
    const int nsteps = a.K / KT;
    const char* xsrc[NIX]; int xoff[NIX];
    const char* wsrc[NIW]; int woff[NIW];
    long wkstride = 0;
#pragma unroll
    for (int it = 0; it < NIX; ++it) {
        const int R0 = (wave * NIX + it) * 16, r = R0 + (lane >> 2), p = lane & 3;
        int gr = m_blk + r; if (gr >= a.M) gr = a.M - 1;
        xsrc[it] = a.X + (long)gr * a.ldx * 2 + ((p ^ swz64(r)) << 4);
        xoff[it] = R0 * ROW64;
    }
    if constexpr (!WT) {
#pragma unroll
        for (int it = 0; it < NIW; ++it) {
            const int R0 = (wave * NIW + it) * 16, r = R0 + (lane >> 2), p = lane & 3;
            int gr = n_blk + r; if (gr >= a.N) gr = a.N - 1;
            wsrc[it] = a.W + (long)gr * a.ldw * 2 + ((p ^ swz64(r)) << 4);
            woff[it] = R0 * ROW64;
        }
    } else {
        const int half = wave >> 1, wq = wave & 1;
        wkstride = a.ldw * 2;
#pragma unroll
        for (int it = 0; it < NIW; ++it) {
            const int R0 = wq * 16 + it * 4, r = R0 + (lane >> 4), p = lane & 15;
            int col = n_blk + half * 128 + ((p ^ swz256(r)) << 3);
            if (col >= a.N) col = 0;
            wsrc[it] = a.W + ((long)r * a.ldw + col) * 2;
            woff[it] = half * KT * 256 + R0 * 256;
        }
    }
    auto issue = [&](int step, int buf) {
        char* xt = xs(buf); char* wt = ws(buf);
#pragma unroll
        for (int it = 0; it < NIX; ++it) glds16_asm(xsrc[it] + (long)step * KT * 2, xt + xoff[it]);
#pragma unroll
        for (int it = 0; it < NIW; ++it) glds16_asm(wsrc[it] + (WT ? (long)step * KT * wkstride : (long)step * KT * 2), wt + woff[it]);
    };
    f32x4 acc[4][WM];
    zero_acc(acc);
#pragma unroll
    for (int p = 0; p < NS - 1; ++p)
        if (p < nsteps) issue(p, p);
    int buf = 0;
    for (int s = 0; s < nsteps; ++s) {
        const int younger = min(NS - 2, nsteps - 1 - s);
        if (younger >= NS - 2) wait_vmcnt<(NS - 2) * LPS>();
        else wait_vmcnt<0>();
        __builtin_amdgcn_s_barrier();
        asm volatile("" ::: "memory");
        if (s + NS - 1 < nsteps) issue(s + NS - 1, buf == 0 ? NS - 1 : buf - 1);
        const char* xt = xs(buf); const char* wt = ws(buf);
        uint4 af[4], bfr[WM];
#pragma unroll
        for (int m = 0; m < 4; ++m) {
            if constexpr (WT) af[m] = frag_tr256(wt + (wn0 >> 7) * KT * 256, (wn0 & 127) + 16 * m, 0);
            else af[m] = frag_sw64(wt, wn0 + 16 * m);
        }
#pragma unroll
        for (int n = 0; n < WM; ++n) bfr[n] = frag_sw64(xt, wm0 + 16 * n);
#pragma unroll
        for (int m = 0; m < 4; ++m)
#pragma unroll
            for (int n = 0; n < WM; ++n) mma_chunk<T>(acc[m][n], af[m], bfr[n]);
        buf = buf + 1 == NS ? 0 : buf + 1;
    }
    if (a.staged >= 0) {
        __syncthreads();
        tile_epilogue_staged<WM>(a, acc, m_blk, n_blk, wm0, wn0, smem, a.staged);
        return;
    }
    tile_epilogue<T, WM, PLAIN>(a, acc, m_blk, n_blk, wm0, wn0, 0);
}
template <bool WT, bool PLAIN>
int launch_wide_p(const GemmArgs& a, hipStream_t st) {
    size_t lds = (size_t)3 * (128 * ROW64 + (WT ? 2 * 32 * 256 : 256 * ROW64));
    if (lds < (size_t)4 * 128 * EPI_LD) lds = (size_t)4 * 128 * EPI_LD;
    FW_SET_LDS_ONCE((gemm_wide_kernel<WT, PLAIN>), lds);
    FW_KNAME("gemm_wide_kernel<%s,%s>", FW_B(WT), FW_B(PLAIN));
    hipLaunchKernelGGL((gemm_wide_kernel<WT, PLAIN>), dim3(fw_cdiv(a.M, 128), fw_cdiv(a.N, 256), 1), dim3(256), lds, st, a);
    FW_LAUNCH_RET();
}

template <bool WT, bool PLAIN>
int launch_big_p(const GemmArgs& a, hipStream_t st) {
    size_t lds = (size_t)2 * (256 * LDS_ROW + (WT ? 2 * 64 * 256 : 256 * LDS_ROW));
    if (lds < (size_t)8 * 128 * EPI_LD) lds = (size_t)8 * 128 * EPI_LD;
    FW_SET_LDS_ONCE((gemm_big_kernel<WT, PLAIN>), lds);
    FW_KNAME("gemm_big_kernel<%s,%s>", FW_B(WT), FW_B(PLAIN));
    hipLaunchKernelGGL((gemm_big_kernel<WT, PLAIN>), dim3(fw_cdiv(a.M, 256), fw_cdiv(a.N, 256), 1), dim3(512), lds, st, a);
    FW_LAUNCH_RET();
}
template <bool WT>
int launch_big(const GemmArgs& a, hipStream_t st) {
    constexpr int BIG_MIN_N = 16384;
    const bool pl = plain_epilogue(a);
    if (a.N >= BIG_MIN_N) return pl ? launch_big_p<WT, true>(a, st) : launch_big_p<WT, false>(a, st);
    return pl ? launch_wide_p<WT, true>(a, st) : launch_wide_p<WT, false>(a, st);
}

#define STREAM_HOT(NCH, EXT) (!((NCH) == 8 && (EXT) != 0))
#define STREAM_MTS(NCH, EXT) 2

template <int NCH, int EXT, int NB>
FW_DEV int stream_hot_strips(const GemmArgs& a, char* smem, const int bnp, const int n_blk, int strip, const int stride, const int full) {
    using T = bf16raw;
    constexpr int MTS = 2, RL = NCH * 64, ROWS = 16 * MTS;
    constexpr int ESZ = EXT == 2 ? 4 : 2;
    static_assert(STREAM_MTS(NCH, EXT) == MTS, "strip height");
    const int l = lane_id(), wave = __builtin_amdgcn_readfirstlane(threadIdx.x >> 6);
    strip = __builtin_amdgcn_readfirstlane(strip);
    const int kbytes = a.K * 2;
    const float* sbias = reinterpret_cast<const float*>(smem + (size_t)bnp * RL);
    struct XSet { uint4 v[MTS][NCH]; };
    struct ESet { uint4 v[MTS][4]; float rs[MTS]; };
    const int ncols = min(bnp, a.N - n_blk);
    unsigned xoff[NCH];
#pragma unroll
    for (int c = 0; c < NCH; ++c) {
        const int kb = c * 64 + ((l >> 4) << 4);
        xoff[c] = (unsigned)(l & 15) * (unsigned)a.ldx * 2u + (unsigned)(kb < kbytes ? kb : 0);
    }
    auto issue_x = [&](XSet& x, int s) {
#pragma unroll
        for (int mt = 0; mt < MTS; ++mt) {
            const char* src = a.X + (long)(s * ROWS + mt * 16) * a.ldx * 2;
#pragma unroll
            for (int c = 0; c < NCH; ++c) x.v[mt][c] = *reinterpret_cast<const uint4*>(src + xoff[c]);
        }
    };
    auto mask_x = [&](XSet& x) {
#pragma unroll
        for (int mt = 0; mt < MTS; ++mt) {
#pragma unroll
            for (int c = 0; c < NCH; ++c) {
                const int valid = kbytes - (c * 64 + ((l >> 4) << 4));
                uint4 v = x.v[mt][c];
                v.x = valid > 0 ? v.x : 0u; v.y = valid > 4 ? v.y : 0u; v.z = valid > 8 ? v.z : 0u; v.w = valid > 12 ? v.w : 0u;
                x.v[mt][c] = v;
            }
        }
    };
    const long lde = EXT == 1 ? a.ldaux : a.ldr;
    const char* ebase = EXT == 1 ? a.aux : reinterpret_cast<const char*>(a.residual);
    auto quad_ok = [&](int j, int i, int l) { return j < NB - 1 || j * 64 + i * 16 + ((l >> 4) << 2) < ncols; };
    auto fetch_e = [&](ESet& e, int s, int j) {
#pragma unroll
        for (int mt = 0; mt < MTS; ++mt) {
            const char* src = ebase + ((long)(s * ROWS + mt * 16) * lde + n_blk + j * 64) * ESZ;
#pragma unroll
            for (int i = 0; i < 4; ++i) {
                const unsigned off = ((unsigned)(l & 15) * (unsigned)lde + (quad_ok(j, i, l) ? (unsigned)(i * 16 + ((l >> 4) << 2)) : 0u)) * ESZ;
                if constexpr (EXT == 1) {
                    const uint2 t = *reinterpret_cast<const uint2*>(src + off);
                    e.v[mt][i].x = t.x; e.v[mt][i].y = t.y;
                } else {
                    e.v[mt][i] = *reinterpret_cast<const uint4*>(src + off);
                }
            }
        }
    };
    const bool has_rs = a.rowscale != nullptr;
    const float* rsp = has_rs ? a.rowscale : a.residual;
    const unsigned rs_div = has_rs ? (unsigned)max(a.rows_per_scale, 1) : 0x80000000u;
    auto fetch_rs = [&](ESet& e, int s) {
#pragma unroll
        for (int mt = 0; mt < MTS; ++mt) e.rs[mt] = rsp[(unsigned)(s * ROWS + mt * 16 + (l & 15)) / rs_div];
    };
    auto pin_x = [&](XSet& x) {
#pragma unroll
// ... 312 lines not shown
                if (nb + 1 < nnb) block(nb + 1, eb, ea);
            }
        } else {
#pragma unroll 1
            for (int nb = 0; nb < nnb; ++nb) {
                f32x4 acc[4][MTS];
                zero_acc(acc);
#pragma unroll
                for (int c = 0; c < NCH; ++c) {
                    uint4 af[4];
#pragma unroll
                    for (int i = 0; i < 4; ++i) {
                        const int row = nb * 64 + i * 16 + (l & 15);
                        af[i] = *reinterpret_cast<const uint4*>(smem + row * RL + ((c * 64 + ((l >> 4) << 4)) ^ swz(row)));
                    }
#pragma unroll
                    for (int i = 0; i < 4; ++i) {
#pragma unroll
                        for (int mt = 0; mt < MTS; ++mt) mma_chunk<T>(acc[i][mt], af[i], xf[mt][c]);
                    }
                }
                if (nb == nnb - 1 && strip + stride < strips) issue_x(strip + stride);
                if constexpr (EXT == 0 && sizeof(T) == 2) {
                    if (a.staged == 0) {
                        char* mine = smem + (size_t)bnp * RL + (size_t)bnp * 4 + wave * (16 * EPI_LD);
                        const int rsub = l >> 3, cb = (l & 7) * 16;
                        const int ncol = n_blk + nb * 64 + (l & 7) * 8;
#pragma unroll
                        for (int mt = 0; mt < MTS; ++mt) {
                            char* rowp = mine + (l & 15) * EPI_LD + ((l >> 4) << 3);
#pragma unroll
                            for (int i = 0; i < 4; ++i) {
                                const f32x4 v = acc[i][mt] + *reinterpret_cast<const f32x4*>(sbias + nb * 64 + i * 16 + ((l >> 4) << 2));
                                *reinterpret_cast<uint2*>(rowp + i * 32) = make_uint2(pack_bf2(v[0], v[1]), pack_bf2(v[2], v[3]));
                            }
                            __builtin_amdgcn_fence(__ATOMIC_RELEASE, "wavefront");
                            asm volatile("s_waitcnt lgkmcnt(0)" ::: "memory");
                            __builtin_amdgcn_fence(__ATOMIC_ACQUIRE, "wavefront");
#pragma unroll
                            for (int it = 0; it < 2; ++it) {
                                const int r = it * 8 + rsub, m = strip * (16 * MTS) + mt * 16 + r;
                                const uint4 v = *reinterpret_cast<const uint4*>(mine + r * EPI_LD + cb);
#ifdef FW_STREAM_DBG
                                if ((a.dbg & 1) && v.x != 0x12345678u) continue;
#endif
                                if (m < a.M && ncol < a.N) *reinterpret_cast<uint4*>(a.C + ((long)m * a.ldc + ncol) * 2) = v;
                            }
                            __builtin_amdgcn_fence(__ATOMIC_RELEASE, "wavefront");
                            asm volatile("s_waitcnt lgkmcnt(0)" ::: "memory");
                            __builtin_amdgcn_fence(__ATOMIC_ACQUIRE, "wavefront");
                        }
                        continue;
                    }
                }
#pragma unroll
                for (int mt = 0; mt < MTS; ++mt) {
                    const int m = m_lane + mt * 16;
                    const int mc = m < a.M ? m : a.M - 1;
                    uint4 ext[4];
                    if constexpr (EXT != 0) {
#pragma unroll
                        for (int i = 0; i < 4; ++i) {
                            const int n0 = n_blk + nb * 64 + i * 16 + ((l >> 4) << 2);
                            epi_fetch<T>(a, ext[i], mc, n0 < a.N ? n0 : 0, 0);
                        }
                    }
#pragma unroll
                    for (int i = 0; i < 4; ++i) {
                        const int n0 = n_blk + nb * 64 + i * 16 + ((l >> 4) << 2);
#ifdef FW_STREAM_DBG
                        if ((a.dbg & 1) && acc[i][mt][0] != 12345.678f) continue;
#endif
                        if (m < a.M && n0 < a.N) epi_apply<T>(a, *reinterpret_cast<const f32x4*>(sbias + (n0 - n_blk)), ext[i], acc[i][mt], m, n0, rs[mt], 0);
                    }
                }
            }
        }
    }
}

template <typename T, int NCH, bool WT, int EXT>
int launch_stream(const GemmArgs& a, hipStream_t st) {
    constexpr int RL = NCH * 64;
    const bool stg = EXT == 0 && sizeof(T) == 2 && a.staged == 0;
    const size_t stage_b = stg ? (size_t)8 * 16 * EPI_LD : 0;
    const int maxb = (int)(((stg ? 60 * 1024 : 64 * 1024)) / RL) & ~63;
    const int ny = fw_cdiv(a.N, maxb);
    const int bnp = fw_cdiv(fw_cdiv(a.N, ny), 64) * 64;
    const size_t lds = (size_t)bnp * RL + (size_t)bnp * 4 + stage_b;
    FW_SET_LDS_ONCE((gemm_stream_kernel<T, NCH, WT, EXT>), 80 * 1024);
    int hot = 0;
    constexpr long LD_MAX = 1L << 24;
    const bool tail16 = a.N % 64 == 0 || a.N % 64 >= 16;
    if (sizeof(T) == 2 && STREAM_HOT(NCH, EXT) && a.alpha == 1.0f && !a.C2 && !a.accumulate && !a.c_zstride && a.ldx < LD_MAX && a.ldc < LD_MAX && a.ldaux < LD_MAX && a.ldr < LD_MAX) {
        if (EXT == 0) hot = stg;
        if (EXT == 1) hot = tail16 && a.act == 2 && !a.out_f32 && !a.rowscale && !a.residual;
        if (EXT == 2) hot = tail16 && a.act == 0 && a.out_f32 && a.residual != nullptr;
    }
#ifdef FW_STREAM_DBG
    if (a.dbg) hot = 0;
#endif
    const int strips = fw_cdiv(a.M, 16 * STREAM_MTS(NCH, EXT));
    int gx = fw_cdiv(strips, 8);
    static const int resident = [] {
        int per_cu = 0, dev = 0;
        hipDeviceProp_t prop;
        if (hipOccupancyMaxActiveBlocksPerMultiprocessor(&per_cu, gemm_stream_kernel<T, NCH, WT, EXT>, 512, 80 * 1024) != hipSuccess || per_cu < 1) per_cu = 1;
        if (hipGetDevice(&dev) != hipSuccess || hipGetDeviceProperties(&prop, dev) != hipSuccess) return 256 * per_cu;
        return prop.multiProcessorCount * per_cu;
    }();
    const int cap = resident / ny > 0 ? resident / ny : 1;
    if (gx > cap) gx = cap;
    FW_KNAME("gemm_stream_kernel<%s,%d,%s,%d>", tname<T>(), NCH, FW_B(WT), EXT);
    hipLaunchKernelGGL((gemm_stream_kernel<T, NCH, WT, EXT>), dim3(gx, ny), dim3(512), lds, st, a, bnp, hot);
    FW_LAUNCH_RET();
}

template <typename T, int NCH>
int dispatch_stream_n(const GemmArgs& a, int wt, hipStream_t st) {
    const int ext = a.act == 2 ? 1 : (a.residual != nullptr ? 2 : 0);
    if (wt) return ext == 1 ? launch_stream<T, NCH, true, 1>(a, st) : ext == 2 ? launch_stream<T, NCH, true, 2>(a, st) : launch_stream<T, NCH, true, 0>(a, st);
    return ext == 1 ? launch_stream<T, NCH, false, 1>(a, st) : ext == 2 ? launch_stream<T, NCH, false, 2>(a, st) : launch_stream<T, NCH, false, 0>(a, st);
}
template <typename T>
int dispatch_stream(const GemmArgs& a, int wt, hipStream_t st) {
    const int nch = fw_cdiv(a.K * TT<T>::SZ, 128) * 2;
    if (nch <= 2) return dispatch_stream_n<T, 2>(a, wt, st);
    if (nch <= 4) return dispatch_stream_n<T, 4>(a, wt, st);
    return dispatch_stream_n<T, 8>(a, wt, st);
}

template <typename T, int BN, bool XT, bool WT, bool GX, bool GW>
int launch(const GemmArgs& a, hipStream_t st) {
    const size_t lds = 2 * (size_t)(BM + BN) * LDS_ROW;
    FW_SET_LDS_ONCE((gemm_kernel<T, BN, XT, WT, GX, GW>), lds);
    dim3 grid(fw_cdiv(a.M, BM), fw_cdiv(a.N, BN), a.splitk);
    FW_KNAME("gemm_kernel<%s,%d,%s,%s,%s,%s>", tname<T>(), BN, FW_B(XT), FW_B(WT), FW_B(GX), FW_B(GW));
    hipLaunchKernelGGL((gemm_kernel<T, BN, XT, WT, GX, GW>), grid, dim3(256), lds, st, a);
    FW_LAUNCH_RET();
}

template <typename T, int BN>
int dispatch_trans(const GemmArgs& a, int xt, int wt, hipStream_t st) {
    const int kt = 128 / TT<T>::SZ;
    const bool whole = a.K % kt == 0;
    const bool gx = !xt && whole && a.x_op == 0, gw = !wt && whole && a.w_op == 0;
    if (!xt && !wt) {
        const int kt64 = 64 / TT<T>::SZ;
        if constexpr (BN == 128) {
            if (a.x_op == 0 && a.w_op == 0 && a.K % kt64 == 0 && !whole) return launch_ring64<T, BN, 3>(a, st);
        }
        if (gx && gw) {
            constexpr int RING3_MIN_STEPS = 28;
            if constexpr (BN == 64) {
                if (a.kper >= RING3_MIN_STEPS * kt) return launch_ring<T, BN, 3>(a, st);
            }
            return launch_ring<T, BN, 2>(a, st);
        }
        if (gx) return launch<T, BN, false, false, true, false>(a, st);
        if (gw) return launch<T, BN, false, false, false, true>(a, st);
        return launch<T, BN, false, false, false, false>(a, st);
    }
    if (!xt && wt) return gx ? launch<T, BN, false, true, true, false>(a, st) : launch<T, BN, false, true, false, false>(a, st);
    if (xt && !wt) return gw ? launch<T, BN, true, false, false, true>(a, st) : launch<T, BN, true, false, false, false>(a, st);
    return launch<T, BN, true, true, false, false>(a, st);
}

}

extern "C" int fw_gemm_last_kernel(char* buf, int n) {
    if (!buf || n <= 0) return -1;
    snprintf(buf, (size_t)n, "%s", g_last_kernel);
    return (int)strlen(g_last_kernel);
}

extern "C" int fw_wgrad_group_prob_bytes(void) { return (int)sizeof(GemmArgs); }
namespace {
__global__ void wgrad_group_fill_kernel(const long long* __restrict__ tab, GemmArgs* __restrict__ probs, int nprob) {
    const int i = blockIdx.x * blockDim.x + threadIdx.x;
    if (i >= nprob) return;
    const long long* t = tab + (size_t)i * 16;
    GemmArgs a;
    a.X = reinterpret_cast<const char*>(t[0]); a.W = reinterpret_cast<const char*>(t[1]); a.C = reinterpret_cast<char*>(t[2]);
    a.ldx = t[3]; a.ldw = t[4]; a.ldc = t[5]; a.M = (int)t[6]; a.N = (int)t[7]; a.K = (int)t[8]; a.kper = (int)t[9]; a.splitk = (int)t[10];
    a.x_op = a.w_op = 0; a.bias = nullptr; a.act = 0; a.slope = 0.f; a.aux = nullptr; a.ldaux = 0; a.rowscale = nullptr; a.rows_per_scale = 1;
    a.residual = nullptr; a.ldr = 0; a.out_f32 = 1; a.accumulate = (int)t[14]; a.C2 = nullptr; a.ldc2 = 0;
    a.xsum = reinterpret_cast<float*>(t[11]); a.c_zstride = t[12]; a.xsum_zstride = t[13]; a.alpha = 1.0f; a.staged = -1; a.dbg = 0;
    probs[i] = a;
}
}
extern "C" int fw_wgrad_group(const void* tab, void* probs, int nprob, const void* items, int nitems, int tile, void* stream) {
    FW_CHECK_ARG(tab && probs && items && nprob > 0 && nitems > 0 && (tile == 128 || tile == 256));
    hipStream_t st = (hipStream_t)stream;
    hipLaunchKernelGGL(wgrad_group_fill_kernel, dim3((nprob + 63) / 64), dim3(64), 0, st, (const long long*)tab, (GemmArgs*)probs, nprob);
    if (tile == 128) {
        const size_t lds = (size_t)3 * (32 * 256 + 32 * 256);
        FW_SET_LDS_ONCE(gemm_wgrad_group_kernel, lds);
        hipLaunchKernelGGL(gemm_wgrad_group_kernel, dim3(nitems), dim3(256), lds, st, (const GemmArgs*)probs, (const int4*)items);
    } else {
        const size_t lds = (size_t)3 * 4 * 32 * 256;
        FW_SET_LDS_ONCE(gemm_wgrad_group_big_kernel, lds);
        hipLaunchKernelGGL(gemm_wgrad_group_big_kernel, dim3(nitems), dim3(512), lds, st, (const GemmArgs*)probs, (const int4*)items);
    }
    FW_LAUNCH_RET();
}

extern "C" int fw_gemm(int dtype, const void* X, long ldx, int x_trans, int x_op, const void* W, long ldw,
                       int w_trans, int w_op, void* C, long ldc, int out_f32, int accumulate, int M, int N,
                       int K, float alpha, const float* bias, int act, float slope, const void* aux,
                       long ldaux, const float* rowscale, int rows_per_scale, const float* residual,
                       long ldr, int splitk, void* C2, long ldc2, float* xsum, long c_zstride, long xsum_zstride,
                       void* stream) {
    const int sz = dtype == FW_DT_BF16 ? 2 : 4;
    const int e16 = 16 / sz;
    FW_CHECK_ARG(dtype == FW_DT_F32 || dtype == FW_DT_BF16);
    FW_CHECK_ARG(M > 0 && N > 0 && K > 0 && X && W && C);
    FW_CHECK_ARG(N % 4 == 0);
    FW_CHECK_ARG(ldx % e16 == 0 && ldw % e16 == 0 && ldc % 4 == 0);
    const int csz = (out_f32 || dtype == FW_DT_F32) ? 4 : 2;
    FW_CHECK_ARG(((uintptr_t)X & 15) == 0 && ((uintptr_t)W & 15) == 0 && ((uintptr_t)C & (4 * csz - 1)) == 0);
    if (!x_trans) FW_CHECK_ARG((K * sz) % 4 == 0 && ldx >= K); else FW_CHECK_ARG(ldx >= M);
    if (!w_trans) FW_CHECK_ARG((K * sz) % 4 == 0 && ldw >= K); else FW_CHECK_ARG(ldw >= N);
    FW_CHECK_ARG(!accumulate || out_f32 || dtype == FW_DT_F32);
    FW_CHECK_ARG(splitk >= 1 && (splitk == 1 || accumulate || c_zstride > 0));
    FW_CHECK_ARG(c_zstride == 0 || (out_f32 && c_zstride % 4 == 0));
    FW_CHECK_ARG(act >= 0 && act <= 3 && (act != 2 || aux));
    FW_CHECK_ARG(!rowscale || rows_per_scale > 0);
    if (bias) FW_CHECK_ARG(((uintptr_t)bias & 15) == 0);
    if (residual) FW_CHECK_ARG(((uintptr_t)residual & 15) == 0 && ldr % 4 == 0);
    const int kt = 128 / sz;
    GemmArgs a;
    a.X = (const char*)X; a.W = (const char*)W; a.C = (char*)C;
    a.ldx = ldx; a.ldw = ldw; a.ldc = ldc; a.M = M; a.N = N; a.K = K;
    a.x_op = x_op; a.w_op = w_op; a.bias = bias; a.act = act; a.slope = slope;
    a.aux = (const char*)aux; a.ldaux = ldaux; a.rowscale = rowscale; a.rows_per_scale = rows_per_scale;
    a.residual = residual; a.ldr = ldr;
    a.out_f32 = (out_f32 || dtype == FW_DT_F32) ? 1 : 0;
    a.accumulate = accumulate;
    a.splitk = splitk;
    a.C2 = (char*)C2; a.ldc2 = ldc2; a.xsum = xsum; a.c_zstride = c_zstride; a.xsum_zstride = xsum_zstride;
    FW_CHECK_ARG(!xsum || x_trans);
    FW_CHECK_ARG(!C2 || (((uintptr_t)C2 & (4 * sz - 1)) == 0 && ldc2 % 4 == 0));
    a.kper = fw_cdiv(fw_cdiv(K, kt), splitk) * kt;
    a.alpha = alpha;
    a.staged = staged_mode(a);
    static const int dbg = getenv("FW_GEMM_BIG_DBG") ? atoi(getenv("FW_GEMM_BIG_DBG")) : 0;
    a.dbg = dbg;
    hipStream_t st = (hipStream_t)stream;
    const bool bf16 = dtype == FW_DT_BF16, no_ops = x_op == 0 && w_op == 0;
    const bool pl = plain_epilogue(a);
    const long tiles128 = (long)fw_cdiv(M, 128) * fw_cdiv(N, 128) * splitk;
    constexpr int STREAM_MIN_M = 32768;
    if (!x_trans && splitk == 1 && !accumulate && no_ops && !xsum && K * sz <= 512 && M >= STREAM_MIN_M)
        return bf16 ? dispatch_stream<bf16raw>(a, w_trans, st) : dispatch_stream<float>(a, w_trans, st);
    constexpr long BIG_MIN_TILES = 160;
    if (bf16 && !x_trans && no_ops && !xsum && splitk == 1 && !accumulate && K % 64 == 0 && K >= 256 &&
        ldx % 8 == 0 && ldw % 8 == 0 && (long)fw_cdiv(M, 256) * fw_cdiv(N, 256) >= BIG_MIN_TILES)
        return w_trans ? launch_big<true>(a, st) : launch_big<false>(a, st);
    const bool tr = bf16 && w_trans && no_ops && (N > 64 || (x_trans && N >= 8)) && K % 64 == 0 && a.kper % 64 == 0 && ldw % 8 == 0;
    if (tr && x_trans && ldx % 8 == 0) return launch_tr_ring<true, 32, 3>(a, st);
    constexpr long TR_MIN_TILES = 200;
    if (tr && !x_trans && !xsum && tiles128 >= TR_MIN_TILES) {
        if (pl && tiles128 > 256) return launch_tr_ring<false, 32, 3>(a, st);
        return pl ? launch_tr_ring<false, 64, 3>(a, st) : launch_tr_ring<false, 64, 2>(a, st);
    }
    constexpr long TR_K32_MIN_TILES = 200;
    if (bf16 && w_trans && !x_trans && no_ops && N > 64 && K % 64 != 0 && K % 32 == 0 && ldw % 8 == 0 && !xsum
        && splitk == 1 && tiles128 >= TR_K32_MIN_TILES)
        return launch_tr_ring<false, 32, 3>(a, st);
    constexpr long BN128_MIN_TILES = 384;
    const bool small_n = N <= 64 || tiles128 < BN128_MIN_TILES;
    if (bf16) return small_n ? dispatch_trans<bf16raw, 64>(a, x_trans, w_trans, st) : dispatch_trans<bf16raw, 128>(a, x_trans, w_trans, st);
    return small_n ? dispatch_trans<float, 64>(a, x_trans, w_trans, st) : dispatch_trans<float, 128>(a, x_trans, w_trans, st);
}
```

frequency-wised_all-in-one_image_restoration_model_amd/fwair/functional.py:

```python
import weakref

import torch

from . import ops
from .lib import call, dt


class config:
    compute_dtype = torch.float32
    shadow_epoch = 0
    direct_grads = False


def act_empty(rows, cols, dtype, device):
    ld = (cols + 7) // 8 * 8
    return torch.empty((rows, ld), dtype=dtype, device=device)[:, :cols]


def aligned(t):
    if t.stride(1) == 1 and (t.stride(0) * t.element_size()) % 16 == 0 and t.data_ptr() % 16 == 0:
        return t
    out = act_empty(t.shape[0], t.shape[1], t.dtype, t.device)
    out.copy_(t)
    return out
# ... 411 lines not shown
        call('fw_attn_fwd', dt(qkv.dtype), D, nkt, lfs, qkv, qkv[:, Cp:], qkv[:, Cp + C:], qkv.stride(0), out, out.stride(0),
             lse, tables, coef, tab, B, H, W, heads, L, mode, shift, float(D) ** -0.5)
        ctx.save_for_backward(qkv, tables, coef, out, lse)
        ctx.geo = geo
        return out

    @staticmethod
    def backward(ctx, dout):
        qkv, tables, coef, out, lse = ctx.saved_tensors
        C, B, H, W, heads, L, mode, shift, lfs = ctx.geo
        D = C // heads
        Cp = (C + 7) // 8 * 8
        rows = qkv.shape[0]
        nkt = 1 if mode == 0 else L - 1
        dout = aligned(dout)
        dqkv = act_empty(rows, qkv.shape[1], qkv.dtype, qkv.device)
        d2 = act_empty(rows, qkv.shape[1], qkv.dtype, qkv.device) if nkt == 2 else None
        tparam, dcoef_to = ctx.side
        if config.direct_grads and tparam is not None and tparam.grad is not None:
            dtab, rtab = tparam.grad.view(tables.shape), None
        else:
            dtab = rtab = _zeros(tables.shape, qkv.device)
        if coef is None:
            dcoef = rcoef = None
        elif dcoef_to is not None:
            dcoef, rcoef = dcoef_to, None
        else:
            dcoef = rcoef = _zeros(coef.shape, qkv.device)
        tab = ops._lfs.device_table(qkv.dtype, qkv.device) if lfs == 2 else None
        call('fw_attn_bwd', dt(qkv.dtype), D, nkt, lfs, qkv, qkv[:, Cp:], qkv[:, Cp + C:], qkv.stride(0), out, out.stride(0),
             dout, dout.stride(0), lse, tables, coef, tab, dqkv, dqkv[:, Cp:], dqkv[:, Cp + C:],
             d2[:, Cp:] if d2 is not None else None, d2[:, Cp + C:] if d2 is not None else None, dqkv.stride(0), dtab, dcoef,
             B, H, W, heads, L, mode, shift, float(D) ** -0.5, Cp - C)
        if nkt == 2:
            call('fw_add_rows', dt(qkv.dtype), d2[:, Cp:], d2.stride(0), dqkv[:, Cp:], dqkv.stride(0), rows, 2 * C)
        dqkv._fw_zero_pad = True
        return dqkv, rtab, rcoef, None, None, None


class DwConvFn(torch.autograd.Function):

    @staticmethod
    def forward(ctx, h1, g1, weight, bias, B, H, W, fuse=None):
        ctx.set_materialize_grads(False)
        C = h1.shape[1]
        wt = shadow(weight, 'dw9')
        if fuse is not None:
            h2, g2 = fuse['h2'], fuse['g2']
        else:
            h2 = act_empty(h1.shape[0], C, h1.dtype, h1.device)
            g2 = act_empty(h1.shape[0], C, h1.dtype, h1.device)
            src = g1 if g1 is not None else h1
            call('fw_dwconv_fwd', dt(h1.dtype), src, src.stride(0), int(g1 is None), wt, bias, h2, g2, h2.stride(0), B, H, W, C)
        if g1 is not None:
            ctx.save_for_backward(h1, weight, wt, g1)
        else:
            ctx.save_for_backward(h1, weight, wt)
        ctx.bias = bias
        ctx.geo = (B, H, W)
        ctx.mark_non_differentiable(g2)
        return h2, g2

    @staticmethod
    def backward(ctx, dh2, _):
        if dh2 is None:
            return (None,) * 8
        h1, weight, wt = ctx.saved_tensors[:3]
        g1 = ctx.saved_tensors[3] if len(ctx.saved_tensors) > 3 else None
        B, H, W = ctx.geo
        C = h1.shape[1]
        dh2 = aligned(dh2)
        db, rb = _grad_target(ctx.bias)
        dw, rw = _grad_target(weight, (C, 9))
        dh1 = act_empty(h1.shape[0], C, h1.dtype, h1.device)
        call('fw_dwconv_bwd', dt(h1.dtype), dh2, dh2.stride(0), g1, h1, h1.stride(0), wt, dh1, dh1.stride(0), dw, db, B, H, W, C)
        return dh1, None, (rw.view_as(weight) if rw is not None else None), rb, None, None, None, None


class DownsampleFn(torch.autograd.Function):

    @staticmethod
    def forward(ctx, x, weight, bias, B, H, W):
        C, Co = x.shape[1], weight.shape[0]
        col = ops.im2col4(x, B, H, W, config.compute_dtype)
        y = torch.empty((col.shape[0], Co), dtype=torch.float32, device=x.device)
        ops.gemm(col, shadow(weight, 'conv4'), col.shape[0], Co, 16 * C, out=y, bias=bias)
        ctx.save_for_backward(x, weight)
        ctx.bias = bias
        ctx.geo = (B, H, W)
        return y

    @staticmethod
    def backward(ctx, dy):
        x, weight = ctx.saved_tensors
        B, H, W = ctx.geo
        C, Co = x.shape[1], weight.shape[0]
        Mo = dy.shape[0]
        g = ops.cast_rows(dy, config.compute_dtype) if config.compute_dtype != torch.float32 else aligned(dy)
        col = ops.im2col4(x, B, H, W, config.compute_dtype)
        dwk = _zeros((Co, 16 * C), x.device)
        db, rb = _grad_target(ctx.bias)
        ops.wgrad(g, col, Co, 16 * C, Mo, dwk, db)
        dw, rw = _grad_target(weight, (Co, C, 16))
        ops.permute3(dwk, dw, (Co, 16, C), (16 * C, 1, 16), accumulate=True)
        del col
        dcol = ops.gemm(g, shadow(weight, 'conv4'), Mo, 16 * C, Co, w_trans=True)
        dx = ops.col2im4(dcol, B, H, W, C)
        return dx, (rw.view_as(weight) if rw is not None else None), rb, None, None, None


class UpsampleCatFn(torch.autograd.Function):

    @staticmethod
    def forward(ctx, x, skip, weight, bias, B, H, W):
        Cin, Cout = weight.shape[0], weight.shape[1]
        Cs = skip.shape[1]
        xq = ops.cast_rows(x, config.compute_dtype) if config.compute_dtype != torch.float32 else x
        g = ops.gemm(xq, shadow(weight, 'convT2'), x.shape[0], 4 * Cout, Cin)
        out = torch.empty((4 * x.shape[0], Cout + Cs), dtype=torch.float32, device=x.device)
        ops.pixel_shuffle(g, bias, out[:, :Cout], B, H, W, Cout)
        ops.copy_rows(skip, out[:, Cout:])
        ctx.save_for_backward(x, weight)
        ctx.bias = bias
        ctx.geo = (B, H, W, Cs)
        return out

    @staticmethod
    def backward(ctx, dcat):
        x, weight = ctx.saved_tensors
        B, H, W, Cs = ctx.geo
        Cin, Cout = weight.shape[0], weight.shape[1]
        M = x.shape[0]
        dg = ops.pixel_unshuffle(dcat[:, :Cout], B, H, W, Cout, config.compute_dtype)
        xq = ops.cast_rows(x, config.compute_dtype) if config.compute_dtype != torch.float32 else x
        dwt = _zeros((4 * Cout, Cin), x.device)
        ops.wgrad(dg, xq, 4 * Cout, Cin, M, dwt)
        dw, rw = _grad_target(weight, (Cin, Cout, 4))
        ops.permute3(dwt, dw, (4, Cout, Cin), (1, 4, Cout * 4), accumulate=True)
        dx = ops.gemm(dg, shadow(weight, 'convT2'), M, Cin, 4 * Cout, w_trans=True, out_dtype=torch.float32)
        db, rb = _grad_target(ctx.bias)
        ops.colsum(dcat[:, :Cout], db)
        dskip = torch.empty((dcat.shape[0], Cs), dtype=torch.float32, device=x.device)
        ops.copy_rows(dcat[:, Cout:], dskip)
        return dx, dskip, (rw.view_as(weight) if rw is not None else None), rb, None, None, None


class InputProjFn(torch.autograd.Function):
    @staticmethod
    def forward(ctx, img, weight, bias):
        B, _, H, W = img.shape
        C = weight.shape[0]
        img = img.contiguous()
        out = torch.empty((B * H * W, C), dtype=torch.float32, device=img.device)
        call('fw_inproj_fwd', img, weight, bias, out, C, B, H, W, C, 0.01)
        ctx.save_for_backward(img, weight, out)
        return out

    @staticmethod
    def backward(ctx, dy):
        img, weight, out = ctx.saved_tensors
        B, _, H, W = img.shape
        C = weight.shape[0]
        dw, db = _zeros(weight.shape, img.device), _zeros((C,), img.device)
        dy = dy.contiguous()
        call('fw_inproj_bwd', img, out, C, dy, dy.stride(0), dw, db, B, H, W, C, 0.01)
        return None, dw, db


class OutputProjFn(torch.autograd.Function):
    @staticmethod
    def forward(ctx, fea, weight, bias, img):
        B, _, H, W = img.shape
        C = fea.shape[1]
        img = img.contiguous()
        out = torch.empty_like(img)
        call('fw_outproj_fwd', fea, fea.stride(0), weight, bias, img, out, B, H, W, C)
        ctx.save_for_backward(fea, weight)
        ctx.geo = (B, H, W)
        return out

    @staticmethod
    def backward(ctx, dout):
        fea, weight = ctx.saved_tensors
        B, H, W = ctx.geo
        C = fea.shape[1]
        dout = dout.contiguous()
        dfea = torch.empty((fea.shape[0], C), dtype=torch.float32, device=fea.device)
        dw, db = _zeros(weight.shape, fea.device), _zeros((3,), fea.device)
        call('fw_outproj_bwd', dout, fea, fea.stride(0), weight, dfea, C, dw, db, B, H, W, C)
        return dfea, dw, db, None


class BnLreluGapFn(torch.autograd.Function):

    @staticmethod
    def forward(ctx, fea, gamma, beta, rmean, rvar, nbt, B, training):
        ED = gamma.shape[0]
        P = fea.numel() // (B * ED)
        assert fea.is_contiguous()
        dev = fea.device
        gap = torch.empty((B, ED), dtype=torch.float32, device=dev)
        part = torch.empty((ED, B, 2), dtype=torch.float32, device=dev) if training else None
        saved = torch.empty((ED, 2), dtype=torch.float32, device=dev) if training else None
        call('fw_bn_lrelu_gap_fwd', dt(fea.dtype), fea, gamma, beta, rmean, rvar, nbt, part, saved, gap, B, ED, P, int(training),
             1e-5, 0.1, 0.1)
        ctx.save_for_backward(fea, gamma, beta, saved)
        ctx.geo = (B, ED, P, training)
        return gap

    @staticmethod
    def backward(ctx, dgap):
        fea, gamma, beta, saved = ctx.saved_tensors
        B, ED, P, training = ctx.geo
        assert training, 'backward through eval-mode BatchNorm is not part of the hot path'
        dev = fea.device
        part2 = torch.empty((ED, B, 2), dtype=torch.float32, device=dev)
        dfea = torch.empty_like(fea)
# ... 320 lines not shown
```

frequency-wised_all-in-one_image_restoration_model_amd/fwair/ops.py:

```python
import bisect

import torch

from . import lfs as _lfs
from .lib import call, dt, lib


def _ld(t):
    assert t.dim() == 2 and t.stride(1) == 1, 'expect a row-major 2-D view'
    return t.stride(0)


def empty(rows, cols, dtype, device):
    return torch.empty((rows, cols), dtype=dtype, device=device)


def gemm(x, w, M, N, K, *, x_trans=False, w_trans=False, x_op=0, w_op=0, out=None, out_dtype=None, bias=None,
         act=0, slope=0.0, aux=None, rowscale=None, rows_per_scale=1, residual=None, accumulate=False, splitk=1,
         alpha=1.0, out_gelu=None, xsum=None, c_zstride=0, xsum_zstride=0):
    assert x.dtype == w.dtype
    if out is None:
        out = torch.empty((M, N), dtype=out_dtype or x.dtype, device=x.device)
    if accumulate:
        _note_write(out)
    if xsum is not None and not xsum_zstride:
        _note_write(xsum)
    out_f32 = int(out.dtype == torch.float32)
    call('fw_gemm', dt(x.dtype), x, _ld(x), int(x_trans), x_op, w, _ld(w), int(w_trans), w_op, out, _ld(out), out_f32,
         int(accumulate), M, N, K, float(alpha), bias, act, float(slope), aux, _ld(aux) if aux is not None else 0,
         rowscale, rows_per_scale, residual, _ld(residual) if residual is not None else 0, splitk,
         out_gelu, _ld(out_gelu) if out_gelu is not None else 0, xsum, c_zstride, xsum_zstride)
    return out


import os as _os
_SPLITK_BLOCKS = int(_os.environ.get('FW_SPLITK_BLOCKS', '512'))
_DGRAD_SPLIT_ROWS = int(_os.environ.get('FW_DGRAD_SPLIT_ROWS', '512'))


def pick_splitk(M, N, K, dtype):
    tiles = ((M + 127) // 128) * ((N + 63) // 64 if N <= 64 else (N + 127) // 128)
    sk = max(1, min(_SPLITK_BLOCKS // max(tiles, 1), K // 512))
    while sk > 1 and sk * M * N * 4 > (256 << 20):
        sk //= 2
    return int(sk)


_zeroed = []
_zeroed_bufs = {}


def _span(t):
    lo = t.data_ptr()
    if t.numel() == 0:
        return lo, lo
    return lo, lo + t.element_size() * (1 + sum((n - 1) * st for n, st in zip(t.shape, t.stride())))


def _clusters(spans):
    order = sorted(range(len(spans)), key=lambda i: spans[i][0])
    union, shared, first = [], [False] * len(spans), 0
    for i in order:
        lo, hi = spans[i]
        if lo >= hi:
            continue
        if union and lo < union[-1][1]:
            union[-1][1] = max(union[-1][1], hi)
            shared[first] = shared[i] = True
        else:
            union.append([lo, hi])
            first = i
    return union, shared


def mark_zeroed(t):
    assert t.is_contiguous()
    lo, hi = _span(t)
    _unmark([(lo, hi)])
    _zeroed.append((lo, hi))
    _zeroed.sort()
    _zeroed_bufs[lo] = t
    for p in [p for p, b in _zeroed_bufs.items() if not any(z[0] < _span(b)[1] and _span(b)[0] < z[1] for z in _zeroed)]:
        del _zeroed_bufs[p]


def clear_marks():
    _zeroed.clear()
    _zeroed_bufs.clear()


def _unmark(spans):
    if not _zeroed or not spans:
        return
    cut, out, j = _clusters(spans)[0], [], 0
    for lo, hi in _zeroed:
        while j < len(cut) and cut[j][1] <= lo:
            j += 1
        cur, k = lo, j
        while k < len(cut) and cut[k][0] < hi:
            if cut[k][0] > cur:
                out.append((cur, cut[k][0]))
            cur = max(cur, cut[k][1])
            k += 1
        if cur < hi:
            out.append((cur, hi))
    _zeroed[:] = out


def _note_write(t):
    if _zeroed and t is not None:
        lo, hi = _span(t)
        i = bisect.bisect_left(_zeroed, (hi,))
        if i and _zeroed[i - 1][1] > lo:
            _unmark([(lo, hi)])
# ... 124 lines not shown
def _groupable(g, x, n, k, m, dw, db):
    return (_GROUP and g.dtype == torch.bfloat16 and x.dtype == torch.bfloat16 and m % 32 == 0 and g.stride(1) == 1 and x.stride(1) == 1
            and g.stride(0) % 8 == 0 and x.stride(0) % 8 == 0 and g.data_ptr() % 16 == 0 and x.data_ptr() % 16 == 0 and n >= 8 and k % 4 == 0
            and dw.dtype == torch.float32 and dw.stride(1) == 1 and dw.stride(0) % 4 == 0 and dw.data_ptr() % 16 == 0)


def _flush_wgrads():
    if not _pending_w:
        return
    work = list(_pending_w)
    _pending_w.clear()
    spans = [_span(w_[5]) for w_ in work]
    shared = _clusters(spans)[1]
    unsliced = [i for i, w_ in enumerate(work) if w_[4] <= _GROUP_CHUNK]
    racing = _clusters([spans[i] for i in unsliced])[1]
    _dw_mode.clear()
    for i, r in zip(unsliced, racing):
        _dw_mode[spans[i]] = 2 if r else 1 if shared[i] or not _GROUP_PLAIN or not _is_zero(spans[i]) else 0
    _unmark(spans + [_span(w_[6]) for w_ in work if w_[6] is not None])
    big = [w for w in work if min(w[2], w[3]) >= _GROUP_BIG_MIN]
    small = [w for w in work if min(w[2], w[3]) < _GROUP_BIG_MIN]
    if big:
        _launch_group(big, 256)
    if small:
        _launch_group(small, 128)


def _group_fire(table, probs, nprob, total, tile):
    call('fw_wgrad_group', table, probs, nprob, table[nprob * 16:], total, tile)


def _launch_group(work, tile=128):
    dev = work[0][0].device
    rows, units = [], []
    for pi, (g, x, n, k, m, dw, db) in enumerate(work):
        tm, tn = (n + tile - 1) // tile, (k + tile - 1) // tile
        sk = max(1, -(-m // _GROUP_CHUNK))
        kper = -(-(-(-m // sk)) // 32) * 32
        sk = -(-m // kper)
        if sk == 1:
            mode = _dw_mode.get(_span(dw), 2)
            rows.append((g.data_ptr(), x.data_ptr(), dw.data_ptr(), g.stride(0), x.stride(0), dw.stride(0), n, k, m, kper, 1,
                         db.data_ptr() if db is not None else 0, 1 if mode == 0 else 0, 0, mode, 0))
        else:
            nk = (n * k + 3) // 4 * 4
            S = nk + (n + 3) // 4 * 4
            slab = torch.empty((sk, S), dtype=torch.float32, device=dev)
            rows.append((g.data_ptr(), x.data_ptr(), slab.data_ptr(), g.stride(0), x.stride(0), k, n, k, m, kper, sk,
                         slab.data_ptr() + 4 * nk if db is not None else 0, S, S if db is not None else 0, 0, 0))
            assert dw.is_contiguous() or dw.stride(0) == k
            _pending.append((slab, sk, n * k, S, dw, db, nk, n if db is not None else 0))
        for z in range(sk):
            for bx in range(0, tm, _GROUP_UNIT_BX):
                units.append((min(kper, m - z * kper), pi, bx, min(_GROUP_UNIT_BX, tm - bx), tn, z))
    units.sort(key=lambda u: -u[0])
    lists, load = [[] for _ in range(8)], [0] * 8
    for ln, pi, bx, u, tn, z in units:
        x = load.index(min(load))
        load[x] += ln * tn * u
        lists[x].extend((pi, bx + i, by, z) for by in range(tn) for i in range(u))
    depth = max(len(li) for li in lists)
    total = depth * 8
    items = [lists[p & 7][p >> 3] if (p >> 3) < len(lists[p & 7]) else (-1, 0, 0, 0) for p in range(total)]
    nprob = len(rows)
    words = nprob * 16 + total * 2
    if words > _HOST_WORDS and len(work) > 1:
        del _pending[len(_pending) - sum(1 for r_ in rows if r_[10] > 1):]
        _launch_group(work[:len(work) // 2], tile); _launch_group(work[len(work) // 2:], tile)
        return
    host = _host_table(words)
    host[:nprob * 16].view(nprob, 16).copy_(torch.tensor(rows, dtype=torch.int64))
    it32 = torch.tensor(items, dtype=torch.int32)
    host[nprob * 16:].view(torch.int32).view(total, 4).copy_(it32)
    table = torch.empty(host.shape, dtype=torch.int64, device=dev)
    table.copy_(host, non_blocking=True)
    probs = torch.empty(nprob * lib().fw_wgrad_group_prob_bytes(), dtype=torch.uint8, device=dev)
    _group_fire(table, probs, nprob, total, tile)
    if not torch.cuda.is_current_stream_capturing():
        for slot in _host_ring:
            if slot[0].data_ptr() == host.data_ptr():
                slot[1].record()


def wgrad(g, x, n, k, m, dw, db=None, defer=False):
    if defer and _in_backward() and _groupable(g, x, n, k, m, dw, db):
        _register_flush()
        _pending_w.append((g, x, n, k, m, dw, db))
        return
    _note_write(dw)
    _note_write(db)
    sk = pick_splitk(n, k, m, g.dtype)
    if sk == 1:
        gemm(g, x, n, k, m, x_trans=True, w_trans=True, out=dw, accumulate=True, xsum=db)
        return
    nk = (n * k + 3) // 4 * 4
    S = nk + (n + 3) // 4 * 4
    slab = torch.empty((sk, S), dtype=torch.float32, device=g.device)
    cview = slab[0, :n * k].view(n, k)
    xs = slab[0, nk:] if db is not None else None
    gemm(g, x, n, k, m, x_trans=True, w_trans=True, out=cview, splitk=sk, xsum=xs, c_zstride=S, xsum_zstride=S if db is not None else 0)
    slab_reduce(slab, sk, n * k, S, dw, db, nk, n, defer=defer)


def dgrad(g, w, M, K, N, out, act=0, aux=None):
    tiles = ((M + 127) // 128) * ((K + 127) // 128)
    sk = min(512 // max(tiles, 1), N // _DGRAD_SPLIT_ROWS) if (act == 0 and tiles < 200) else 1
    if sk <= 1:
        gemm(g, w, M, K, N, w_trans=True, out=out, act=act, aux=aux)
        return
    S = (M * K + 3) // 4 * 4
    slab = torch.empty((sk, S), dtype=torch.float32, device=g.device)
    gemm(g, w, M, K, N, w_trans=True, out=slab[0, :M * K].view(M, K), splitk=sk, c_zstride=S)
    direct = out.dtype == torch.float32 and out.is_contiguous()
    tmp = out if direct else torch.empty((M, K), dtype=torch.float32, device=g.device)
    call('fw_slab_reduce', slab, sk, M * K, S, tmp, 0, None, 0, 0)
    if not direct:
        call('fw_cast_rows', dt(out.dtype), tmp, K, out, _ld(out), M, K, None, 1)


def layernorm_fwd(x, gamma, beta, out_dtype, eps=1e-5):
    rows, C = x.shape
    y = torch.empty((rows, C), dtype=out_dtype, device=x.device)
    mean = torch.empty(rows, dtype=torch.float32, device=x.device)
    rstd = torch.empty(rows, dtype=torch.float32, device=x.device)
    call('fw_layernorm_fwd', dt(out_dtype), x, _ld(x), gamma, beta, y, _ld(y), mean, rstd, rows, C, eps)
    return y, mean, rstd


def layernorm_bwd(dy, x, gamma, mean, rstd, dgamma, dbeta, dres=None, defer=False, twin=None, twscale=None, tw_rows_per_scale=1):
    rows, C = x.shape
    dx = torch.empty((rows, C), dtype=torch.float32, device=x.device)
    nblk = lib().fw_layernorm_bwd_blocks(rows, C)
    partial = torch.empty((nblk, 2 * C), dtype=torch.float32, device=x.device)
    call('fw_layernorm_bwd2', dt(dy.dtype), dy, _ld(dy), x, _ld(x), gamma, mean, rstd, dres,
         _ld(dres) if dres is not None else 0, dx, _ld(dx), None, None, partial, rows, C,
         twin, _ld(twin) if twin is not None else 0, twscale, tw_rows_per_scale)
    slab_reduce(partial, nblk, C, 2 * C, dgamma, dbeta, C, C, defer=defer)
    return dx


def layernorm_mod_fwd(x, gamma, beta, mod, H, W, shift, y, eps=1e-5):
    rows, C = x.shape
    mean = torch.empty(rows, dtype=torch.float32, device=x.device)
    rstd = torch.empty(rows, dtype=torch.float32, device=x.device)
    call('fw_layernorm_mod_fwd', dt(y.dtype), x, _ld(x), gamma, beta, mod, y, _ld(y), mean, rstd, rows, C, H, W, shift, eps)
    return mean, rstd


def modulator_bwd(dy, dmod, H, W, shift, defer=False):
    rows, C = dy.shape
    nz = lib().fw_modulator_bwd_blocks(rows, C)
    partial = torch.empty((nz, 64 * C), dtype=torch.float32, device=dy.device)
    deferred = defer and _in_backward()
    if not deferred:
        _note_write(dmod)
    call('fw_modulator_bwd', dt(dy.dtype), dy, _ld(dy), None if deferred else dmod, partial, rows, C, H, W, shift)
    if deferred:
        slab_reduce(partial, nz, 64 * C, 64 * C, dmod, defer=True)


def attn_fwd(qkv, C, B, H, W, heads, L, mode, shift, bias, coef=None, lfs=0):
    rows = qkv.shape[0]
    D = C // heads
    nkt = 1 if mode == 0 else L - 1
    out = torch.empty((rows, C), dtype=qkv.dtype, device=qkv.device)
    nitems = B * (H // 8) * (W // 8) * L * heads
    lse = torch.empty((nitems, 64), dtype=torch.float32, device=qkv.device)
    tab = _lfs.device_table(qkv.dtype, qkv.device) if lfs == 2 else None
    call('fw_attn_fwd', dt(qkv.dtype), D, nkt, lfs, qkv, qkv[:, C:], qkv[:, 2 * C:], _ld(qkv), out, _ld(out), lse, bias,
         coef, tab, B, H, W, heads, L, mode, shift, float(D) ** -0.5)
    return out, lse


def attn_bwd(qkv, out, dout, lse, C, B, H, W, heads, L, mode, shift, bias, dbias_dense, coef=None, dcoef=None, lfs=0):
    rows = qkv.shape[0]
    D = C // heads
    nkt = 1 if mode == 0 else L - 1
    dqkv = torch.empty_like(qkv)
    d2 = torch.empty_like(qkv) if nkt == 2 else None
    _note_write(dbias_dense)
    _note_write(dcoef)
    tab = _lfs.device_table(qkv.dtype, qkv.device) if lfs == 2 else None
    call('fw_attn_bwd', dt(qkv.dtype), D, nkt, lfs, qkv, qkv[:, C:], qkv[:, 2 * C:], _ld(qkv), out, _ld(out), dout, _ld(dout),
         lse, bias, coef, tab, dqkv, dqkv[:, C:], dqkv[:, 2 * C:], d2[:, C:] if d2 is not None else None,
         d2[:, 2 * C:] if d2 is not None else None, _ld(dqkv),
         dbias_dense, dcoef, B, H, W, heads, L, mode, shift, float(D) ** -0.5, 0)
    if nkt == 2:
        call('fw_add_rows', dt(qkv.dtype), d2[:, C:], _ld(d2), dqkv[:, C:], _ld(dqkv), rows, 2 * C)
    return dqkv


def rel_index(device):
    ch = torch.arange(8)
    coords = torch.stack(torch.meshgrid([ch, ch], indexing='ij')).flatten(1)
    rel = (coords[:, :, None] - coords[:, None, :]).permute(1, 2, 0).contiguous()
    rel[:, :, 0] += 7
    rel[:, :, 1] += 7
    rel[:, :, 0] *= 15
    return rel.sum(-1).to(device)


def dwconv_fwd(src, w, bias, B, H, W, in_gelu=False):
    h2, g2 = torch.empty_like(src), torch.empty_like(src)
    call('fw_dwconv_fwd', dt(src.dtype), src, _ld(src), int(in_gelu), w, bias, h2, g2, _ld(h2), B, H, W, src.shape[1])
    return h2, g2


def dwconv_bwd(dh2, g1, h1, w, dw, dbias, B, H, W):
    dh1 = torch.empty_like(h1)
    _note_write(dw)
    _note_write(dbias)
    call('fw_dwconv_bwd', dt(h1.dtype), dh2, _ld(dh2), g1, h1, _ld(h1), w, dh1, _ld(dh1), dw, dbias, B, H, W, h1.shape[1])
    return dh1


def im2col4(x, B, H, W, dtype):
    C = x.shape[1]
    col = torch.empty((B * (H // 2) * (W // 2), 16 * C), dtype=dtype, device=x.device)
    call('fw_im2col4', dt(dtype), x, _ld(x), col, B, H, W, C)
    return col


def col2im4(dcol, B, H, W, C, dres=None):
    dx = torch.empty((B * H * W, C), dtype=torch.float32, device=dcol.device)
    call('fw_col2im4', dt(dcol.dtype), dcol, dx, _ld(dx), dres, _ld(dres) if dres is not None else 0, B, H, W, C)
    return dx


def pixel_shuffle(g, bias, out, B, H, W, Cout):
    call('fw_pixel_shuffle', dt(g.dtype), g, bias, out, _ld(out), B, H, W, Cout)
    return out


def pixel_unshuffle(dout, B, H, W, Cout, dtype):
    dg = torch.empty((B * H * W, 4 * Cout), dtype=dtype, device=dout.device)
    call('fw_pixel_unshuffle', dt(dtype), dout, _ld(dout), dg, B, H, W, Cout)
    return dg


def colsum(x, out):
    _note_write(out)
    call('fw_colsum', 1 if x.dtype == torch.bfloat16 else 0, x, _ld(x), out, x.shape[0], x.shape[1])


def cast_rows(src, dtype, rowscale=None, rows_per_scale=1):
    dst = torch.empty(src.shape, dtype=dtype, device=src.device)
    call('fw_cast_rows', dt(dtype), src, _ld(src), dst, _ld(dst), src.shape[0], src.shape[1], rowscale, rows_per_scale)
    return dst


def copy_rows(src, dst, accumulate=False):
    if accumulate:
        _note_write(dst)
    call('fw_copy_rows', src, _ld(src), dst, _ld(dst), src.shape[0], src.shape[1], int(accumulate))


def permute3(src, dst, dims, out_strides, accumulate=False):
    ind = 1 if src.dtype == torch.bfloat16 else 0
    outd = 1 if dst.dtype == torch.bfloat16 else 0
    if accumulate:
        _note_write(dst)
    call('fw_permute3', ind, outd, src, dst, dims[0], dims[1], dims[2], out_strides[0], out_strides[1], out_strides[2],
         int(accumulate))
```

include/fwair.h:

```cpp
#ifndef FWAIR_H
#define FWAIR_H
#ifdef __cplusplus
extern "C" {
#endif

int fw_gemm(int dtype, const void* X, long ldx, int x_trans, int x_op, const void* W, long ldw, int w_trans, int w_op,
            void* C, long ldc, int out_f32, int accumulate, int M, int N, int K, float alpha, const float* bias, int act,
            float slope, const void* aux, long ldaux, const float* rowscale, int rows_per_scale, const float* residual,
            long ldr, int splitk, void* C2, long ldc2, float* xsum, long c_zstride, long xsum_zstride, void* stream);
int fw_gemm_last_kernel(char* buf, int n);

int fw_wgrad_group_prob_bytes(void);
int fw_wgrad_group(const void* tab, void* probs, int nprob, const void* items, int nitems, int tile, void* stream);

int fw_slab_reduce(const float* slab, int nz, long n, long zstride, float* dst, int accumulate, float* dst2, long off2, long n2,
                   void* stream);
int fw_slab_reduce_multi(const void* tab, const void* prefix, int num, long total_blocks, void* stream);

int fw_layernorm_fwd(int dtype, const float* x, long ldx, const float* gamma, const float* beta, void* y, long ldy,
                     float* mean, float* rstd, int rows, int C, float eps, void* stream);
int fw_layernorm_bwd_blocks(int rows, int C);
int fw_layernorm_bwd(int dtype, const void* dy, long lddy, const float* x, long ldx, const float* gamma, const float* mean,
                     const float* rstd, const float* dres, long lddres, float* dx, long lddx, float* dgamma, float* dbeta,
                     float* partial, int rows, int C, void* stream);
int fw_layernorm_bwd2(int dtype, const void* dy, long lddy, const float* x, long ldx, const float* gamma, const float* mean,
                      const float* rstd, const float* dres, long lddres, float* dx, long lddx, float* dgamma, float* dbeta,
                      float* partial, int rows, int C, void* twin, long ldtw, const float* twscale, int tw_rows_per_scale,
                      void* stream);

int fw_layernorm_mod_fwd(int dtype, const float* x, long ldx, const float* gamma, const float* beta, const float* mod, void* y,
                         long ldy, float* mean, float* rstd, int rows, int C, int H, int W, int shift, float eps, void* stream);
int fw_modulator_bwd_blocks(int rows, int C);
int fw_modulator_bwd(int dtype, const void* dy, long lddy, float* dmod, float* partial, int rows, int C, int H, int W, int shift,
                     void* stream);

int fw_attn_lfs_table_elems(void);
int fw_attn_fwd(int dtype, int D, int nkt, int lfs, const void* q, const void* k, const void* v, long ld, void* out, long ldo,
                float* lse, const float* bias, const float* coef, const void* lfs_tab, int B, int H, int W, int heads, int L,
                int mode, int shift, float scale, void* stream);
int fw_attn_bwd(int dtype, int D, int nkt, int lfs, const void* q, const void* k, const void* v, long ld, const void* out,
                long ldo, const void* dout, long lddo, const float* lse, const float* bias, const float* coef,
                const void* lfs_tab, void* dq, void* dk, void* dv, void* dk2, void* dv2, long ldd, float* dbias,
                float* dcoef, int B, int H, int W, int heads, int L, int mode, int shift, float scale, int dq_pad, void* stream);

int fw_dwconv_fwd(int dtype, const void* in, long ld1, int in_gelu, const float* w, const float* bias, void* h2, void* g2, long ld2, int B,
                  int H, int W, int C, void* stream);
int fw_dwconv_bwd(int dtype, const void* dh2, long ldg, const void* g1, const void* h1, long ld1, const float* w, void* dh1,
                  long ldo, float* dw, float* dbias, int B, int H, int W, int C, void* stream);

int fw_im2col4(int dtype, const float* x, long ldx, void* col, int B, int H, int W, int C, void* stream);
int fw_col2im4(int dtype, const void* dcol, float* dx, long lddx, const float* dres, long ldr, int B, int H, int W, int C,
               void* stream);
int fw_pixel_shuffle(int dtype, const void* g, const float* bias, float* out, long ldo, int B, int H, int W, int Cout,
                     void* stream);
int fw_pixel_unshuffle(int dtype, const float* dout, long ldo, void* dg, int B, int H, int W, int Cout, void* stream);
int fw_colsum(int x_dtype, const void* x, long ldx, float* out, long rows, int cols, void* stream);

int fw_inproj_fwd(const float* img, const float* w, const float* bias, float* out, long ldo, int B, int H, int W, int C,
                  float slope, void* stream);
int fw_inproj_bwd(const float* img, const float* out, long ldo, const float* dy, long ldy, float* dw, float* db, int B, int H,
                  int W, int C, float slope, void* stream);
int fw_outproj_fwd(const float* fea, long ldf, const float* w, const float* bias, const float* img, float* out, int B, int H,
                   int W, int C, void* stream);
int fw_outproj_bwd(const float* dout, const float* fea, long ldf, const float* w, float* dfea, long lddf, float* dw, float* db,
                   int B, int H, int W, int C, void* stream);

int fw_cast_rows(int dtype, const float* src, long lds_, void* dst, long ldd, long rows, int cols, const float* rowscale,
                 int rows_per_scale, void* stream);
int fw_copy_rows(const float* src, long lds_, float* dst, long ldd, long rows, int cols, int accumulate, void* stream);
int fw_add_rows(int dtype, const void* src, long lds_, void* dst, long ldd, long rows, int cols, void* stream);
int fw_cast_flat(int dtype, const float* src, void* dst, long n, void* stream);
int fw_permute3(int in_dtype, int out_dtype, const void* in, void* out, int d0, int d1, int d2, long s0, long s1, long s2,
                int accumulate, void* stream);
int fw_permute3_multi(const void* tab, const void* prefix, int num, long total_blocks, void* stream);
int fw_fill(float* p, long n, float v, void* stream);
int fw_lrelu_fwd(int dtype, const float* x, void* y, long n, float slope, void* stream);
int fw_lrelu_bwd(int dtype, const void* dy, const float* x, float* dx, long n, float slope, void* stream);

int fw_l1_loss(const float* a, const float* b, float* da, long n, float gscale, float* loss, void* stream);
int fw_ce0_loss(const float* logits, float* dlogits, int R, int N, float gscale, float* loss, void* stream);

int fw_adam_tick(float* hyper, float b1, float b2, void* stream);
int fw_adam(int shadow_dtype, float* p, const float* g, float* m, float* v, void* shadow, long n, const float* hyper, float b1,
            float b2, float eps, void* stream);
int fw_ema(int shadow_dtype, float* pk, const float* pq, void* shadow, long n, float momentum, void* stream);

int fw_dft2_fwd(const float* img, float* fr, float* fi, int nimg, int N, void* stream);
int fw_dft2_bands(const float* fr, const float* fi, const float* mask_unshifted, float* out, int nimg, int N, int nbands,
                  int mode, void* stream);
int fw_dft2_decompose(const float* img, const float* mask, const float* panels, float* out, int nimg, int N, int nbands, int dc_bits,
                      void* stream);
int fw_band_residual(const float* img, float* out, int nimg, int N, int nbands, void* stream);
int fw_dc_split(const float* img, float* out, int nimg, int NN, void* stream);
int fw_dft2t_fwd(const float* img, const float* panels, float* work, float* fr, float* fi, int nimg, int N, void* stream);
int fw_dft2t_bands(const float* fr, const float* fi, const float* mask_unshifted, const float* panels, float* work, float* out,
                   int nimg, int N, int nbands, int mode, void* stream);
int fw_dft2t_decompose(const float* img, const float* mask, const float* panels, float* work, float* out, int nimg, int N,
                       int nbands, int dc_bits, void* stream);
int fw_band_stats(int src_kind, const void* src, const unsigned char* clean, const unsigned char* ring, const float* panels_h,
                  const float* panels_w, float* work, double* out, int nimg, int H, int W, int nbands, int power, void* stream);
int fw_band_split(int src_kind, const void* src, const unsigned char* clean, const unsigned char* ring, const float* panels_h,
                  const float* panels_w, float* work, float* out, int nimg, int H, int W, int nbands, int mode, void* stream);

int fw_bn_lrelu_gap_fwd(int dtype, const void* fea, const float* gamma, const float* beta, float* rmean, float* rvar,
                        long long* nbt, float* part, float* saved, float* gap, int B, int ED, int P, int training, float eps,
                        float momentum, float slope, void* stream);
int fw_bn_lrelu_gap_bwd(int dtype, const void* fea, const float* gamma, const float* beta, const float* saved, const float* dgap,
                        float* part2, void* dfea, float* dgamma, float* dbeta, int B, int ED, int P, float slope, void* stream);

int fw_moco_logits(const float* q, const float* k, const float* queue, float* logits, float* khat, int L, int B, int ED, int K,
                   float invT, void* stream);
int fw_moco_logits_bwd(const float* q, const float* khat, const float* queue, const float* dlogits, float* dq, int L, int B,
                       int ED, int K, float invT, void* stream);
int fw_moco_enqueue(float* queue, const float* khat, long long* ptr, int L, int B, int ED, int K, void* stream);

int fw_lfs_xbar(const float* inter, float* xbar, float* stats, int nb1, int B, int NT, int C, float eps, void* stream);
int fw_lfs_xbar_bwd(const float* inter, const float* stats, const float* dxbar, float* dinter, int nb1, int B, int NT, int C,
                    void* stream);
int fw_lfs_lambda(const float* xbar, const unsigned long long* ptab, const int* heads, const long long* coef_off, float* coef,
                  float* save, int nblk, int B, int C, int nb1, void* stream);
int fw_lfs_lambda_bwd(const float* xbar, const unsigned long long* ptab, const unsigned long long* gtab, const int* heads,
                      const long long* coef_off, const float* dcoef, const float* save, float* dxbar, int nblk, int B, int C,
                      int nb1, void* stream);

int fw_conv3x3(int dtype, const void* x, long ldx, const void* x2, long ldx2, int cin, int cin1, const void* w, const float* bias,
               void* out, long ldo, int out_f32, const void* res, long ldr, int cout, int B, int H, int W, int stride, int taps,
               int act, float slope, void* stream);
int fw_im2col3(int dtype, const void* x, long ldx, void* col, int B, int H, int W, int C, int stride, void* stream);
int fw_col2im3(int dtype, const void* dcol, void* dx, long lddx, int B, int H, int W, int C, int stride, void* stream);
int fw_dcn_im2col(int dtype, const void* x, long ldx, const float* om, void* col, int B, int H, int W, int C, void* stream);
int fw_dcn_bwd(int dtype, const void* dcol, const void* x, long ldx, const float* om, float* dx, long lddx, float* dom, int B, int H,
               int W, int C, void* stream);
int fw_bn_cl_fwd(int dtype, const void* x, long ldx, const float* gamma, const float* beta, float* rmean, float* rvar, long long* nbt,
                 float* sums, float* mr, const void* res, long ldr, void* y, long ldy, long rows, int C, int training, float eps,
                 float momentum, float slope, void* stream);
// ... 74 lines not shown
```

Before: 341.8 images/sec.

## Replace conv4 im2col with implicit-gather GEMM over padded bf16 input

The 4x4 stride-2 downsample conv no longer builds an explicit im2col buffer in forward and again in backward. It pads and casts the input once to bf16 and has the GEMM and weight-grad kernels compute gather addresses on the fly using magic-number division, then saves the padded tensor for backward. This cuts the large 16x-expanded column buffer traffic and the duplicated im2col in backward. The cost is more address arithmetic and less contiguous global-to-LDS loads inside the GEMM. It also makes the upsample path save the already-cast input so backward skips a cast.

```diff
diff --git a/frequency-wised_all-in-one_image_restoration_model_amd/csrc/fw_common.h b/frequency-wised_all-in-one_image_restoration_model_amd/csrc/fw_common.h
--- a/frequency-wised_all-in-one_image_restoration_model_amd/csrc/fw_common.h
+++ b/frequency-wised_all-in-one_image_restoration_model_amd/csrc/fw_common.h
@@ -245,7 +245,43 @@
     FW_MEM void mac(f32x4 (&acc)[2][2]) const { mac(acc, acc); }
 };
 
-#define FW_CHECK_ARG(cond)                                                                   \
+#define FW_HD static __host__ __device__ __forceinline__
+struct Conv4Geo {
+    int Ho, Wo;
+    int seg, seggap;
+    long rs_b; int rs_y, rs_x;
+    unsigned long long mul_wo, mul_hw;
+    int sh_wo, sh_hw;
+};
+FW_HD unsigned conv4_div(unsigned t, unsigned long long mul, int sh) { return (unsigned)(((unsigned long long)t * mul) >> sh); }
+FW_HD long conv4_row_off(const Conv4Geo& g, unsigned t) {
+    const unsigned t2 = conv4_div(t, g.mul_wo, g.sh_wo), b = conv4_div(t, g.mul_hw, g.sh_hw);
+    const int ox = (int)(t - t2 * (unsigned)g.Wo), oy = (int)(t2 - b * (unsigned)g.Ho);
+    return (long)b * g.rs_b + (oy * g.rs_y + ox * g.rs_x);
+}
+FW_HD int conv4_k_off(const Conv4Geo& g, int k) {
+    const int ky = (k >= g.seg) + (k >= 2 * g.seg) + (k >= 3 * g.seg);
+    return k + ky * g.seggap;
+}
+static inline void conv4_magic(unsigned d, unsigned long long* mul, int* sh) {
+    int L = 0;
+    while ((1ull << L) < d) ++L;
+    *sh = 32 + L;
+    *mul = ((1ull << (32 + L)) + d - 1) / d;
+}
+static inline bool conv4_geo_make(Conv4Geo* g, int B, int H, int W, int C) {
+    if (B < 1 || H < 2 || W < 2 || C < 4 || (H & 1) || (W & 1) || (C & 3)) return false;
+    const long img = (long)(H + 2) * (W + 2) * C, ntok = (long)B * (H / 2) * (W / 2);
+    if (img >= (1L << 30) || ntok >= (1L << 31)) return false;
+    g->Ho = H / 2; g->Wo = W / 2;
+    g->seg = 4 * C; g->seggap = (W + 2) * C - 4 * C;
+    g->rs_b = img; g->rs_y = 2 * (W + 2) * C; g->rs_x = 2 * C;
+    conv4_magic((unsigned)g->Wo, &g->mul_wo, &g->sh_wo);
+    conv4_magic((unsigned)(g->Ho * g->Wo), &g->mul_hw, &g->sh_hw);
+    return true;
+}
+
+#define FW_CHECK_ARG(cond)                                                                  \
     do {                                                                                     \
         if (!(cond)) return -__LINE__;                                                       \
     } while (0)
diff --git a/frequency-wised_all-in-one_image_restoration_model_amd/csrc/fw_elem.hip b/frequency-wised_all-in-one_image_restoration_model_amd/csrc/fw_elem.hip
--- a/frequency-wised_all-in-one_image_restoration_model_amd/csrc/fw_elem.hip
+++ b/frequency-wised_all-in-one_image_restoration_model_amd/csrc/fw_elem.hip
@@ -818,6 +818,38 @@
 #pragma unroll
             for (int e = 0; e < 4; ++e) acc[e] = ok[k] ? acc[e] + f[k][e] : acc[e];
         *reinterpret_cast<f32x4*>(dx + (long)tok * lddx + c) = acc;
+    }
+}
+
+constexpr int PC4_PIECES = 4;
+__global__ __launch_bounds__(256) void pad_cast4_kernel(const float* __restrict__ x, long ldx, uint4* __restrict__ xpad, int B, int H, int W, int C,
+                                                        unsigned npieces) {
+    const unsigned c4n = (unsigned)C >> 2, Wp = (unsigned)W + 2, Hp = (unsigned)H + 2;
+    f32x4 v[PC4_PIECES][2];
+    bool ok[PC4_PIECES][2];
+#pragma unroll
+    for (int i = 0; i < PC4_PIECES; ++i) {
+        unsigned q = (blockIdx.x * PC4_PIECES + i) * 256u + threadIdx.x;
+        if (q >= npieces) q = npieces - 1;
+        unsigned pix = (2u * q) / c4n, cg = 2u * q - pix * c4n;
+        unsigned px = pix % Wp, t = pix / Wp, py = t % Hp, b = t / Hp;
+#pragma unroll
+        for (int h = 0; h < 2; ++h) {
+            ok[i][h] = px >= 1 && px <= (unsigned)W && py >= 1 && py <= (unsigned)H;
+            const unsigned sx = min(max(px, 1u), (unsigned)W) - 1, sy = min(max(py, 1u), (unsigned)H) - 1;
+            v[i][h] = *reinterpret_cast<const f32x4*>(x + (((long)b * H + sy) * W + sx) * ldx + cg * 4);
+            if (++cg == c4n) {
+                cg = 0;
+                if (++px == Wp) { px = 0; if (++py == Hp) { py = 0; ++b; } }
+            }
+        }
+    }
+#pragma unroll
+    for (int i = 0; i < PC4_PIECES; ++i) {
+        const unsigned q = (blockIdx.x * PC4_PIECES + i) * 256u + threadIdx.x;
+        const f32x4 z = f32x4{0.f, 0.f, 0.f, 0.f};
+        const f32x4 lo = ok[i][0] ? v[i][0] : z, hi = ok[i][1] ? v[i][1] : z;
+        if (q < npieces) xpad[q] = make_uint4(pack_bf2(lo[0], lo[1]), pack_bf2(lo[2], lo[3]), pack_bf2(hi[0], hi[1]), pack_bf2(hi[2], hi[3]));
     }
 }
 
@@ -1489,6 +1521,16 @@
     if (dtype == FW_DT_BF16) LAUNCH((col2im4_kernel<bf16raw>), n, (const bf16raw*)dcol, dx, lddx, dres, ldr, B, H, W, C);
     LAUNCH((col2im4_kernel<float>), n, (const float*)dcol, dx, lddx, dres, ldr, B, H, W, C);
 }
+extern "C" int fw_pad_cast4(const float* x, long ldx, void* xpad, int B, int H, int W, int C, void* stream) {
+    FW_CHECK_ARG(x && xpad && B > 0 && H >= 2 && W >= 2 && C >= 4 && C % 4 == 0 && H % 2 == 0 && W % 2 == 0 && ldx >= C && ldx % 4 == 0);
+    FW_CHECK_ARG(((uintptr_t)x & 15) == 0 && ((uintptr_t)xpad & 15) == 0);
+    const long groups = (long)B * (H + 2) * (W + 2) * (C / 4);
+    FW_CHECK_ARG(groups < (1L << 31));
+    const unsigned npieces = (unsigned)(groups / 2);
+    hipLaunchKernelGGL(pad_cast4_kernel, dim3((npieces + 256 * PC4_PIECES - 1) / (256 * PC4_PIECES)), dim3(256), 0, ST, x, ldx, (uint4*)xpad, B, H, W, C,
+                       npieces);
+    FW_LAUNCH_RET();
+}
 extern "C" int fw_pixel_shuffle(int dtype, const void* g, const float* bias, float* out, long ldo, int B, int H, int W, int Cout,
                                 void* stream) {
     FW_CHECK_ARG(g && bias && out && Cout % 4 == 0 && ldo % 4 == 0);
diff --git a/frequency-wised_all-in-one_image_restoration_model_amd/csrc/fw_gemm.hip b/frequency-wised_all-in-one_image_restoration_model_amd/csrc/fw_gemm.hip
--- a/frequency-wised_all-in-one_image_restoration_model_amd/csrc/fw_gemm.hip
+++ b/frequency-wised_all-in-one_image_restoration_model_amd/csrc/fw_gemm.hip
@@ -2,6 +2,7 @@
 #include <stdio.h>
 #include <string.h>
 #include <stdlib.h>
+#include <type_traits>
 
 namespace {
 static thread_local char g_last_kernel[96] = "";
@@ -28,6 +29,8 @@
     float alpha;
     int staged;
     int dbg;
+    int gather;
+    Conv4Geo geo;
 };
 
 constexpr int LDS_ROW = 128;
@@ -600,6 +603,51 @@
     }
 };
 
+template <int ROWS> struct GldsKcConv4 {
+    static constexpr int NI = ROWS / 32;
+    const char* rowp[NI];
+    int ke[NI], loff[NI];
+    FW_MEM void init(const char* base, const Conv4Geo& g, int row0, int rows_total, int k0) {
+        const int lane = threadIdx.x & 63, wave = threadIdx.x >> 6;
+#pragma unroll
+        for (int it = 0; it < NI; ++it) {
+            const int R0 = (wave * NI + it) * 8;
+            const int r = R0 + (lane >> 3), p = lane & 7;
+            int gr = row0 + r;
+            if (gr >= rows_total) gr = rows_total - 1;
+            rowp[it] = base + conv4_row_off(g, (unsigned)gr) * 2;
+            ke[it] = k0 + ((p ^ (swz(r) >> 4)) << 3);
+            loff[it] = R0 * LDS_ROW;
+        }
+    }
+    FW_MEM void issue(int step, char* tile, const Conv4Geo& g) const {
+#pragma unroll
+        for (int it = 0; it < NI; ++it) glds16_asm(rowp[it] + conv4_k_off(g, ke[it] + step * 64) * 2, tile + loff[it]);
+    }
+};
+template <int KT> struct GldsKmConv4 {
+    static constexpr int NI = KT / 16;
+    const char* colp[NI];
+    int tok[NI], loff[NI];
+    FW_MEM void init(const char* base, const Conv4Geo& g, int col0, int cols_total, int k0) {
+        const int lane = threadIdx.x & 63, wave = threadIdx.x >> 6;
+#pragma unroll
+        for (int it = 0; it < NI; ++it) {
+            const int R0 = wave * (KT / 4) + it * 4;
+            const int r = R0 + (lane >> 4), p = lane & 15;
+            int col = col0 + ((p ^ swz256(r)) << 3);
+            if (col >= cols_total) col = 0;
+            colp[it] = base + (long)conv4_k_off(g, col) * 2;
+            tok[it] = k0 + r;
+            loff[it] = R0 * 256;
+        }
+    }
+    FW_MEM void issue(int step, char* tile, const Conv4Geo& g) const {
+#pragma unroll
+        for (int it = 0; it < NI; ++it) glds16_asm(colp[it] + conv4_row_off(g, (unsigned)(tok[it] + step * KT)) * 2, tile + loff[it]);
+    }
+};
+
 constexpr int ROW64 = 64;
 FW_DEV int swz64(int r) { return (r >> 2) & 3; }
 template <typename T, int ROWS> struct GldsKc64 {
@@ -702,7 +750,7 @@
     return -1;
 }
 
-template <bool XT, int KT, int NS, bool PLAIN>
+template <bool XT, int KT, int NS, bool PLAIN, bool GA = false>
 FW_DEV void tr_ring_tile(const GemmArgs& a, int bx, int by, int bz, char* smem) {
     using T = bf16raw;
     static_assert(NS == 2 || NS == 3, "ring depth");
@@ -726,8 +774,9 @@
     const bool do_xsum = XT && a.xsum != nullptr && by == 0 && wn0 == 0;
     const uint4 ones = make_uint4(0x3F803F80u, 0x3F803F80u, 0x3F803F80u, 0x3F803F80u);
 
-    GldsKm<KT> gw;
-    gw.init(a.W, a.ldw, n_blk, a.N, k_begin);
+    std::conditional_t<GA, GldsKmConv4<KT>, GldsKm<KT>> gw;
+    if constexpr (GA) gw.init(a.W, a.geo, n_blk, a.N, k_begin);
+    else gw.init(a.W, a.ldw, n_blk, a.N, k_begin);
     GldsKm<XT ? KT : 16> gxm;
     GldsKc<T, BM> gxc;
     GldsKc64<T, BM> gxc64;
@@ -738,7 +787,8 @@
         if constexpr (XT) gxm.issue(step, xs(buf));
         else if constexpr (X64) gxc64.issue(step, xs(buf));
         else gxc.issue(step, xs(buf));
-        gw.issue(step, ws(buf));
+        if constexpr (GA) gw.issue(step, ws(buf), a.geo);
+        else gw.issue(step, ws(buf));
     };
 #pragma unroll
     for (int p = 0; p < NS - 1; ++p)
@@ -812,6 +862,30 @@
     }
     tr_ring_tile<XT, KT, NS, PLAIN>(a, bx, by, bz, smem);
 }
+template <bool PLAIN>
+__global__ __launch_bounds__(256, 3) void gemm_tr_ring_conv4_kernel(GemmArgs a) {
+    extern __shared__ __attribute__((aligned(16))) char smem[];
+    int bx = blockIdx.x, by = blockIdx.y, bz = blockIdx.z;
+    {
+        const unsigned total = gridDim.x * gridDim.y * gridDim.z;
+        if (gridDim.z > 1) {
+            const unsigned lin = blockIdx.x + gridDim.x * (blockIdx.y + gridDim.y * blockIdx.z);
+            const unsigned w = xcd_contiguous(lin, total);
+            bx = (int)(w % gridDim.x);
+            by = (int)((w / gridDim.x) % gridDim.y);
+            bz = (int)(w / (gridDim.x * gridDim.y));
+        } else if (gridDim.z == 1 && gridDim.y > 1) {
+            const unsigned lin = blockIdx.x + gridDim.x * blockIdx.y;
+            const unsigned w = xcd_contiguous(lin, total);
+            const unsigned per_band = 8 * gridDim.y;
+            const unsigned band = w / per_band, first = band * 8;
+            const unsigned gsz = min(gridDim.x - first, 8u);
+            bx = (int)(first + (w % per_band) % gsz);
+            by = (int)((w % per_band) / gsz);
+        }
+    }
+    tr_ring_tile<true, 32, 3, PLAIN, true>(a, bx, by, bz, smem);
+}
 
 __global__ __launch_bounds__(256, 3) void gemm_wgrad_group_kernel(const GemmArgs* __restrict__ probs, const int4* __restrict__ items) {
     extern __shared__ __attribute__((aligned(16))) char smem[];
@@ -923,6 +997,14 @@
     const size_t lds = (size_t)NS * ((XT ? KT * 256 : 128 * ((KT == 32) ? ROW64 : LDS_ROW)) + KT * 256);
     FW_SET_LDS_ONCE((gemm_tr_ring_kernel<XT, KT, NS, PLAIN>), lds);
     FW_KNAME("gemm_tr_ring_kernel<%s,%d,%d,%s>", FW_B(XT), KT, NS, FW_B(PLAIN));
+    if constexpr (XT && KT == 32 && NS == 3) {
+        if (a.gather == 2) {
+            FW_SET_LDS_ONCE((gemm_tr_ring_conv4_kernel<PLAIN>), lds);
+            hipLaunchKernelGGL((gemm_tr_ring_conv4_kernel<PLAIN>), dim3(fw_cdiv(a.M, 128), fw_cdiv(a.N, 128), a.splitk), dim3(256), lds, st, a);
+            FW_LAUNCH_RET();
+        }
+    }
+    if (a.gather) return -__LINE__;
     hipLaunchKernelGGL((gemm_tr_ring_kernel<XT, KT, NS, PLAIN>), dim3(fw_cdiv(a.M, 128), fw_cdiv(a.N, 128), a.splitk), dim3(256), lds, st, a);
     FW_LAUNCH_RET();
 }
@@ -1012,12 +1094,100 @@
     tile_epilogue<T, WM, PLAIN>(a, acc, m_blk, n_blk, wm0, wn0, bz);
 }
 
+template <int BN, int NS>
+__global__ __launch_bounds__(256) void gemm_ring_conv4_kernel(GemmArgs a) {
+    using T = bf16raw;
+    constexpr int KT = 64;
+    constexpr int WM = (BN == 128) ? 4 : 2;
+    constexpr int XBYTES = BM * LDS_ROW, WBYTES = BN * LDS_ROW, STAGE = XBYTES + WBYTES;
+    constexpr int LPS = BM / 32 + BN / 32;
+    extern __shared__ __attribute__((aligned(16))) char smem[];
+    auto xs = [&](int i) -> char* { return smem + i * STAGE; };
+    auto ws = [&](int i) -> char* { return smem + i * STAGE + XBYTES; };
+    const int wave = threadIdx.x >> 6;
+    int bx = blockIdx.x, by = blockIdx.y, bz = blockIdx.z;
+    {
+        const unsigned total = gridDim.x * gridDim.y * gridDim.z;
+        if (gridDim.z > 1) {
+            const unsigned lin = blockIdx.x + gridDim.x * (blockIdx.y + gridDim.y * blockIdx.z);
+            const unsigned w = xcd_contiguous(lin, total);
+            bx = (int)(w % gridDim.x);
+            by = (int)((w / gridDim.x) % gridDim.y);
+            bz = (int)(w / (gridDim.x * gridDim.y));
+        } else if (gridDim.z == 1 && gridDim.y > 1) {
+            const unsigned lin = blockIdx.x + gridDim.x * blockIdx.y;
+            const unsigned w = xcd_contiguous(lin, total);
+            const unsigned per_band = 8 * gridDim.y;
+            const unsigned band = w / per_band, first = band * 8;
+            const unsigned gsz = min(gridDim.x - first, 8u);
+            bx = (int)(first + (w % per_band) % gsz);
+            by = (int)((w % per_band) / gsz);
+        }
+    }
+    const int m_blk = bx * BM, n_blk = by * BN;
+    const int wm0 = (BN == 128) ? (wave & 1) * 64 : wave * 32;
+    const int wn0 = (BN == 128) ? (wave >> 1) * 64 : 0;
+    const int k_begin = bz * a.kper;
+    const int k_end = min(a.K, k_begin + a.kper);
+    const int nsteps = (k_end - k_begin) / KT;
+
+    f32x4 acc[4][WM];
+    zero_acc(acc);
+    GldsKcConv4<BM> gx;
+    GldsKc<T, BN> gw;
+    gx.init(a.X, a.geo, m_blk, a.M, k_begin);
+    gw.init(a.W, a.ldw, n_blk, a.N, k_begin * TT<T>::SZ);
+    auto issue = [&](int step, int buf) {
+        gx.issue(step, xs(buf), a.geo);
+        gw.issue(step, ws(buf));
+    };
+#pragma unroll
+    for (int p = 0; p < NS - 1; ++p)
+        if (p < nsteps) issue(p, p);
+    int buf = 0;
+    for (int s = 0; s < nsteps; ++s) {
+        const int younger = min(NS - 2, nsteps - 1 - s);
+        if (younger >= NS - 2) wait_vmcnt<(NS - 2) * LPS>();
+        else wait_vmcnt<0>();
+        __builtin_amdgcn_s_barrier();
+        asm volatile("" ::: "memory");
+        if (s + NS - 1 < nsteps) issue(s + NS - 1, buf == 0 ? NS - 1 : buf - 1);
+#pragma unroll
+        for (int c = 0; c < 2; ++c) {
+            uint4 af[4], bfr[WM];
+#pragma unroll
+            for (int m = 0; m < 4; ++m) af[m] = frag_sw(ws(buf), wn0 + 16 * m, c);
+#pragma unroll
+            for (int n = 0; n < WM; ++n) bfr[n] = frag_sw(xs(buf), wm0 + 16 * n, c);
+#pragma unroll
+            for (int m = 0; m < 4; ++m)
+#pragma unroll
+                for (int n = 0; n < WM; ++n) mma_chunk<T>(acc[m][n], af[m], bfr[n]);
+        }
+        buf = buf + 1 == NS ? 0 : buf + 1;
+    }
+    if (a.staged >= 0 && (size_t)NS * STAGE >= (size_t)4 * 16 * WM * EPI_LD) {
+        __syncthreads();
+        tile_epilogue_staged<WM>(a, acc, m_blk, n_blk, wm0, wn0, smem, a.staged);
+        return;
+    }
+    tile_epilogue<T, WM, true>(a, acc, m_blk, n_blk, wm0, wn0, bz);
+}
+
 template <typename T, int BN, int NS, bool PLAIN>
 int launch_ring_p(const GemmArgs& a, hipStream_t st) {
     const size_t lds = (size_t)NS * (BM + BN) * LDS_ROW;
-    FW_SET_LDS_ONCE((gemm_ring_kernel<T, BN, NS, PLAIN>), lds);
     dim3 grid(fw_cdiv(a.M, BM), fw_cdiv(a.N, BN), a.splitk);
     FW_KNAME("gemm_ring_kernel<%s,%d,%d,%s>", tname<T>(), BN, NS, FW_B(PLAIN));
+    if constexpr (sizeof(T) == 2 && PLAIN) {
+        if (a.gather == 1) {
+            FW_SET_LDS_ONCE((gemm_ring_conv4_kernel<BN, NS>), lds);
+            hipLaunchKernelGGL((gemm_ring_conv4_kernel<BN, NS>), grid, dim3(256), lds, st, a);
+            FW_LAUNCH_RET();
+        }
+    }
+    if (a.gather) return -__LINE__;
+    FW_SET_LDS_ONCE((gemm_ring_kernel<T, BN, NS, PLAIN>), lds);
     hipLaunchKernelGGL((gemm_ring_kernel<T, BN, NS, PLAIN>), grid, dim3(256), lds, st, a);
     FW_LAUNCH_RET();
 }
@@ -1109,6 +1279,7 @@
 template <typename T, int BN, int NS, bool PLAIN>
 int launch_ring64_p(const GemmArgs& a, hipStream_t st) {
     const size_t lds = (size_t)NS * (BM + BN) * ROW64;
+    if (a.gather) return -__LINE__;
     FW_SET_LDS_ONCE((gemm_ring64_kernel<T, BN, NS, PLAIN>), lds);
     dim3 grid(fw_cdiv(a.M, BM), fw_cdiv(a.N, BN), a.splitk);
     FW_KNAME("gemm_ring64_kernel<%s,%d,%d,%s>", tname<T>(), BN, NS, FW_B(PLAIN));
@@ -1223,13 +1394,12 @@
     tile_epilogue<T, WM, PLAIN>(a, acc, m_blk, n_blk, wm0, wn0, 0);
 }
 
-template <bool WT, bool PLAIN>
-__global__ __launch_bounds__(256, 2) void gemm_wide_kernel(GemmArgs a) {
+template <bool WT, bool PLAIN, bool GA>
+FW_DEV void wide_tile(const GemmArgs& a, char* smem) {
     using T = bf16raw;
     constexpr int KT = 32, NS = 3, WM = 8, TM = 128, TN = 256;
     constexpr int XB = TM * ROW64, WB = WT ? 2 * KT * 256 : TN * ROW64, STAGE = XB + WB;
     constexpr int NIX = 2, NIW = 4, LPS = NIX + NIW;
-    extern __shared__ __attribute__((aligned(16))) char smem[];
     auto xs = [&](int i) -> char* { return smem + i * STAGE; };
     auto ws = [&](int i) -> char* { return smem + i * STAGE + XB; };
     const int lane = threadIdx.x & 63, wave = threadIdx.x >> 6;
@@ -1248,13 +1418,15 @@
     const int wm0 = 0, wn0 = wave * 64;
     const int nsteps = a.K / KT;
     const char* xsrc[NIX]; int xoff[NIX];
+    int xke[GA ? NIX : 1];
     const char* wsrc[NIW]; int woff[NIW];
     long wkstride = 0;
 #pragma unroll
     for (int it = 0; it < NIX; ++it) {
         const int R0 = (wave * NIX + it) * 16, r = R0 + (lane >> 2), p = lane & 3;
         int gr = m_blk + r; if (gr >= a.M) gr = a.M - 1;
-        xsrc[it] = a.X + (long)gr * a.ldx * 2 + ((p ^ swz64(r)) << 4);
+        if constexpr (GA) { xsrc[it] = a.X + conv4_row_off(a.geo, (unsigned)gr) * 2; xke[it] = (p ^ swz64(r)) << 3; }
+        else xsrc[it] = a.X + (long)gr * a.ldx * 2 + ((p ^ swz64(r)) << 4);
         xoff[it] = R0 * ROW64;
     }
     if constexpr (!WT) {
@@ -1280,7 +1452,10 @@
     auto issue = [&](int step, int buf) {
         char* xt = xs(buf); char* wt = ws(buf);
 #pragma unroll
-        for (int it = 0; it < NIX; ++it) glds16_asm(xsrc[it] + (long)step * KT * 2, xt + xoff[it]);
+        for (int it = 0; it < NIX; ++it) {
+            if constexpr (GA) glds16_asm(xsrc[it] + conv4_k_off(a.geo, xke[it] + step * KT) * 2, xt + xoff[it]);
+            else glds16_asm(xsrc[it] + (long)step * KT * 2, xt + xoff[it]);
+        }
 #pragma unroll
         for (int it = 0; it < NIW; ++it) glds16_asm(wsrc[it] + (WT ? (long)step * KT * wkstride : (long)step * KT * 2), wt + woff[it]);
     };
@@ -1320,11 +1495,28 @@
     tile_epilogue<T, WM, PLAIN>(a, acc, m_blk, n_blk, wm0, wn0, 0);
 }
 template <bool WT, bool PLAIN>
+__global__ __launch_bounds__(256, 2) void gemm_wide_kernel(GemmArgs a) {
+    extern __shared__ __attribute__((aligned(16))) char smem[];
+    wide_tile<WT, PLAIN, false>(a, smem);
+}
+__global__ __launch_bounds__(256, 2) void gemm_wide_conv4_kernel(GemmArgs a) {
+    extern __shared__ __attribute__((aligned(16))) char smem[];
+    wide_tile<false, true, true>(a, smem);
+}
+template <bool WT, bool PLAIN>
 int launch_wide_p(const GemmArgs& a, hipStream_t st) {
     size_t lds = (size_t)3 * (128 * ROW64 + (WT ? 2 * 32 * 256 : 256 * ROW64));
     if (lds < (size_t)4 * 128 * EPI_LD) lds = (size_t)4 * 128 * EPI_LD;
+    FW_KNAME("gemm_wide_kernel<%s,%s>", FW_B(WT), FW_B(PLAIN));
+    if constexpr (!WT && PLAIN) {
+        if (a.gather == 1) {
+            FW_SET_LDS_ONCE(gemm_wide_conv4_kernel, lds);
+            hipLaunchKernelGGL(gemm_wide_conv4_kernel, dim3(fw_cdiv(a.M, 128), fw_cdiv(a.N, 256), 1), dim3(256), lds, st, a);
+            FW_LAUNCH_RET();
+        }
+    }
+    if (a.gather) return -__LINE__;
     FW_SET_LDS_ONCE((gemm_wide_kernel<WT, PLAIN>), lds);
-    FW_KNAME("gemm_wide_kernel<%s,%s>", FW_B(WT), FW_B(PLAIN));
     hipLaunchKernelGGL((gemm_wide_kernel<WT, PLAIN>), dim3(fw_cdiv(a.M, 128), fw_cdiv(a.N, 256), 1), dim3(256), lds, st, a);
     FW_LAUNCH_RET();
 }
@@ -1333,6 +1525,7 @@
 int launch_big_p(const GemmArgs& a, hipStream_t st) {
     size_t lds = (size_t)2 * (256 * LDS_ROW + (WT ? 2 * 64 * 256 : 256 * LDS_ROW));
     if (lds < (size_t)8 * 128 * EPI_LD) lds = (size_t)8 * 128 * EPI_LD;
+    if (a.gather) return -__LINE__;
     FW_SET_LDS_ONCE((gemm_big_kernel<WT, PLAIN>), lds);
     FW_KNAME("gemm_big_kernel<%s,%s>", FW_B(WT), FW_B(PLAIN));
     hipLaunchKernelGGL((gemm_big_kernel<WT, PLAIN>), dim3(fw_cdiv(a.M, 256), fw_cdiv(a.N, 256), 1), dim3(512), lds, st, a);
@@ -1811,6 +2004,7 @@
 template <typename T, int NCH, bool WT, int EXT>
 int launch_stream(const GemmArgs& a, hipStream_t st) {
     constexpr int RL = NCH * 64;
+    if (a.gather) return -__LINE__;
     const bool stg = EXT == 0 && sizeof(T) == 2 && a.staged == 0;
     const size_t stage_b = stg ? (size_t)8 * 16 * EPI_LD : 0;
     const int maxb = (int)(((stg ? 60 * 1024 : 64 * 1024)) / RL) & ~63;
@@ -1862,6 +2056,7 @@
 template <typename T, int BN, bool XT, bool WT, bool GX, bool GW>
 int launch(const GemmArgs& a, hipStream_t st) {
     const size_t lds = 2 * (size_t)(BM + BN) * LDS_ROW;
+    if (a.gather) return -__LINE__;
     FW_SET_LDS_ONCE((gemm_kernel<T, BN, XT, WT, GX, GW>), lds);
     dim3 grid(fw_cdiv(a.M, BM), fw_cdiv(a.N, BN), a.splitk);
     FW_KNAME("gemm_kernel<%s,%d,%s,%s,%s,%s>", tname<T>(), BN, FW_B(XT), FW_B(WT), FW_B(GX), FW_B(GW));
@@ -1915,6 +2110,7 @@
     a.x_op = a.w_op = 0; a.bias = nullptr; a.act = 0; a.slope = 0.f; a.aux = nullptr; a.ldaux = 0; a.rowscale = nullptr; a.rows_per_scale = 1;
     a.residual = nullptr; a.ldr = 0; a.out_f32 = 1; a.accumulate = (int)t[14]; a.C2 = nullptr; a.ldc2 = 0;
     a.xsum = reinterpret_cast<float*>(t[11]); a.c_zstride = t[12]; a.xsum_zstride = t[13]; a.alpha = 1.0f; a.staged = -1; a.dbg = 0;
+    a.gather = 0; a.geo = Conv4Geo{};
     probs[i] = a;
 }
 }
@@ -1934,14 +2130,31 @@
     FW_LAUNCH_RET();
 }
 
-extern "C" int fw_gemm(int dtype, const void* X, long ldx, int x_trans, int x_op, const void* W, long ldw,
-                       int w_trans, int w_op, void* C, long ldc, int out_f32, int accumulate, int M, int N,
-                       int K, float alpha, const float* bias, int act, float slope, const void* aux,
-                       long ldaux, const float* rowscale, int rows_per_scale, const float* residual,
-                       long ldr, int splitk, void* C2, long ldc2, float* xsum, long c_zstride, long xsum_zstride,
-                       void* stream) {
+static int gemm_entry(int dtype, const void* X, long ldx, int x_trans, int x_op, const void* W, long ldw,
+                      int w_trans, int w_op, void* C, long ldc, int out_f32, int accumulate, int M, int N,
+                      int K, float alpha, const float* bias, int act, float slope, const void* aux,
+                      long ldaux, const float* rowscale, int rows_per_scale, const float* residual,
+                      long ldr, int splitk, void* C2, long ldc2, float* xsum, long c_zstride, long xsum_zstride,
+                      int gather, int gB, int gH, int gW, int gC, void* stream) {
     const int sz = dtype == FW_DT_BF16 ? 2 : 4;
     const int e16 = 16 / sz;
+    Conv4Geo geo = Conv4Geo{};
+    if (gather) {
+        FW_CHECK_ARG(gather == 1 || gather == 2);
+        FW_CHECK_ARG(dtype == FW_DT_BF16 && x_op == 0 && w_op == 0);
+        FW_CHECK_ARG(conv4_geo_make(&geo, gB, gH, gW, gC));
+        const long ntok = (long)gB * geo.Ho * geo.Wo;
+        FW_CHECK_ARG(conv4_row_off(geo, (unsigned)(ntok - 1)) % 8 == 0 && conv4_k_off(geo, 16 * gC - 8) % 8 == 0);
+        if (gather == 1) {
+            FW_CHECK_ARG(!x_trans && !w_trans && K == 16 * gC && M == ntok && ldx == gC);
+            FW_CHECK_ARG(splitk == 1 && !accumulate && !xsum && c_zstride == 0);
+            FW_CHECK_ARG(act == 0 && !rowscale && !residual && !C2 && alpha == 1.0f);
+            ldx = K;
+        } else {
+            FW_CHECK_ARG(x_trans && w_trans && N == 16 * gC && K == ntok && ldw == gC);
+            ldw = N;
+        }
+    }
     FW_CHECK_ARG(dtype == FW_DT_F32 || dtype == FW_DT_BF16);
     FW_CHECK_ARG(M > 0 && N > 0 && K > 0 && X && W && C);
     FW_CHECK_ARG(N % 4 == 0);
@@ -1975,6 +2188,7 @@
     a.staged = staged_mode(a);
     static const int dbg = getenv("FW_GEMM_BIG_DBG") ? atoi(getenv("FW_GEMM_BIG_DBG")) : 0;
     a.dbg = dbg;
+    a.gather = gather; a.geo = geo;
     hipStream_t st = (hipStream_t)stream;
     const bool bf16 = dtype == FW_DT_BF16, no_ops = x_op == 0 && w_op == 0;
     const bool pl = plain_epilogue(a);
@@ -2002,3 +2216,37 @@
     if (bf16) return small_n ? dispatch_trans<bf16raw, 64>(a, x_trans, w_trans, st) : dispatch_trans<bf16raw, 128>(a, x_trans, w_trans, st);
     return small_n ? dispatch_trans<float, 64>(a, x_trans, w_trans, st) : dispatch_trans<float, 128>(a, x_trans, w_trans, st);
 }
+
+extern "C" int fw_gemm(int dtype, const void* X, long ldx, int x_trans, int x_op, const void* W, long ldw,
+                       int w_trans, int w_op, void* C, long ldc, int out_f32, int accumulate, int M, int N,
+                       int K, float alpha, const float* bias, int act, float slope, const void* aux,
+                       long ldaux, const float* rowscale, int rows_per_scale, const float* residual,
+                       long ldr, int splitk, void* C2, long ldc2, float* xsum, long c_zstride, long xsum_zstride,
+                       void* stream) {
+    return gemm_entry(dtype, X, ldx, x_trans, x_op, W, ldw, w_trans, w_op, C, ldc, out_f32, accumulate, M, N, K, alpha, bias, act, slope,
+                      aux, ldaux, rowscale, rows_per_scale, residual, ldr, splitk, C2, ldc2, xsum, c_zstride, xsum_zstride, 0, 0, 0, 0, 0, stream);
+}
+extern "C" int fw_gemm_conv4(int dtype, const void* X, long ldx, int x_trans, int x_op, const void* W, long ldw,
+                             int w_trans, int w_op, void* C, long ldc, int out_f32, int accumulate, int M, int N,
+                             int K, float alpha, const float* bias, int act, float slope, const void* aux,
+                             long ldaux, const float* rowscale, int rows_per_scale, const float* residual,
+                             long ldr, int splitk, void* C2, long ldc2, float* xsum, long c_zstride, long xsum_zstride,
+                             int B, int H, int W_, int C_, int gather, void* stream) {
+    FW_CHECK_ARG(gather == 1 || gather == 2);
+    return gemm_entry(dtype, X, ldx, x_trans, x_op, W, ldw, w_trans, w_op, C, ldc, out_f32, accumulate, M, N, K, alpha, bias, act, slope,
+                      aux, ldaux, rowscale, rows_per_scale, residual, ldr, splitk, C2, ldc2, xsum, c_zstride, xsum_zstride, gather, B, H, W_, C_,
+                      stream);
+}
+extern "C" int fw_conv4_offsets(int B, int H, int W, int C, long t0, int n, long* row_off) {
+    Conv4Geo g;
+    FW_CHECK_ARG(row_off && n >= 0 && t0 >= 0 && conv4_geo_make(&g, B, H, W, C));
+    FW_CHECK_ARG(t0 + n <= (long)B * g.Ho * g.Wo);
+    for (int i = 0; i < n; ++i) row_off[i] = conv4_row_off(g, (unsigned)(t0 + i));
+    return 0;
+}
+extern "C" int fw_conv4_k_offsets(int B, int H, int W, int C, int k0, int n, long* k_off) {
+    Conv4Geo g;
+    FW_CHECK_ARG(k_off && n >= 0 && k0 >= 0 && conv4_geo_make(&g, B, H, W, C) && k0 + n <= 16 * C);
+    for (int i = 0; i < n; ++i) k_off[i] = conv4_k_off(g, k0 + i);
+    return 0;
+}
diff --git a/frequency-wised_all-in-one_image_restoration_model_amd/fwair/functional.py b/frequency-wised_all-in-one_image_restoration_model_amd/fwair/functional.py
--- a/frequency-wised_all-in-one_image_restoration_model_amd/fwair/functional.py
+++ b/frequency-wised_all-in-one_image_restoration_model_amd/fwair/functional.py
@@ -517,10 +517,17 @@
     @staticmethod
     def forward(ctx, x, weight, bias, B, H, W):
         C, Co = x.shape[1], weight.shape[0]
-        col = ops.im2col4(x, B, H, W, config.compute_dtype)
-        y = torch.empty((col.shape[0], Co), dtype=torch.float32, device=x.device)
-        ops.gemm(col, shadow(weight, 'conv4'), col.shape[0], Co, 16 * C, out=y, bias=bias)
-        ctx.save_for_backward(x, weight)
+        Mo = B * (H // 2) * (W // 2)
+        ctx.gather = (B, H, W, C) if ops.conv4_gather_ok(B, H, W, C, config.compute_dtype) else None
+        y = torch.empty((Mo, Co), dtype=torch.float32, device=x.device)
+        if ctx.gather:
+            xpad = ops.pad_cast4(x, B, H, W)
+            ops.gemm(xpad, shadow(weight, 'conv4'), Mo, Co, 16 * C, out=y, bias=bias, gather=ctx.gather)
+            ctx.save_for_backward(xpad, weight)
+        else:
+            col = ops.im2col4(x, B, H, W, config.compute_dtype)
+            ops.gemm(col, shadow(weight, 'conv4'), Mo, Co, 16 * C, out=y, bias=bias)
+            ctx.save_for_backward(x, weight)
         ctx.bias = bias
         ctx.geo = (B, H, W)
         return y
@@ -532,10 +539,10 @@
         C, Co = x.shape[1], weight.shape[0]
         Mo = dy.shape[0]
         g = ops.cast_rows(dy, config.compute_dtype) if config.compute_dtype != torch.float32 else aligned(dy)
-        col = ops.im2col4(x, B, H, W, config.compute_dtype)
+        col = x if ctx.gather else ops.im2col4(x, B, H, W, config.compute_dtype)
         dwk = _zeros((Co, 16 * C), x.device)
         db, rb = _grad_target(ctx.bias)
-        ops.wgrad(g, col, Co, 16 * C, Mo, dwk, db)
+        ops.wgrad(g, col, Co, 16 * C, Mo, dwk, db, gather=ctx.gather)
         dw, rw = _grad_target(weight, (Co, C, 16))
         ops.permute3(dwk, dw, (Co, 16, C), (16 * C, 1, 16), accumulate=True)
         del col
@@ -555,19 +562,19 @@
         out = torch.empty((4 * x.shape[0], Cout + Cs), dtype=torch.float32, device=x.device)
         ops.pixel_shuffle(g, bias, out[:, :Cout], B, H, W, Cout)
         ops.copy_rows(skip, out[:, Cout:])
-        ctx.save_for_backward(x, weight)
+        ctx.save_for_backward(xq, weight)
         ctx.bias = bias
         ctx.geo = (B, H, W, Cs)
         return out
 
     @staticmethod
     def backward(ctx, dcat):
-        x, weight = ctx.saved_tensors
+        xq, weight = ctx.saved_tensors
+        x = xq
         B, H, W, Cs = ctx.geo
         Cin, Cout = weight.shape[0], weight.shape[1]
         M = x.shape[0]
         dg = ops.pixel_unshuffle(dcat[:, :Cout], B, H, W, Cout, config.compute_dtype)
-        xq = ops.cast_rows(x, config.compute_dtype) if config.compute_dtype != torch.float32 else x
         dwt = _zeros((4 * Cout, Cin), x.device)
         ops.wgrad(dg, xq, 4 * Cout, Cin, M, dwt)
         dw, rw = _grad_target(weight, (Cin, Cout, 4))
diff --git a/frequency-wised_all-in-one_image_restoration_model_amd/fwair/ops.py b/frequency-wised_all-in-one_image_restoration_model_amd/fwair/ops.py
--- a/frequency-wised_all-in-one_image_restoration_model_amd/fwair/ops.py
+++ b/frequency-wised_all-in-one_image_restoration_model_amd/fwair/ops.py
@@ -17,7 +17,7 @@
 
 def gemm(x, w, M, N, K, *, x_trans=False, w_trans=False, x_op=0, w_op=0, out=None, out_dtype=None, bias=None,
          act=0, slope=0.0, aux=None, rowscale=None, rows_per_scale=1, residual=None, accumulate=False, splitk=1,
-         alpha=1.0, out_gelu=None, xsum=None, c_zstride=0, xsum_zstride=0):
+         alpha=1.0, out_gelu=None, xsum=None, c_zstride=0, xsum_zstride=0, gather=None):
     assert x.dtype == w.dtype
     if out is None:
         out = torch.empty((M, N), dtype=out_dtype or x.dtype, device=x.device)
@@ -26,10 +26,14 @@
     if xsum is not None and not xsum_zstride:
         _note_write(xsum)
     out_f32 = int(out.dtype == torch.float32)
-    call('fw_gemm', dt(x.dtype), x, _ld(x), int(x_trans), x_op, w, _ld(w), int(w_trans), w_op, out, _ld(out), out_f32,
-         int(accumulate), M, N, K, float(alpha), bias, act, float(slope), aux, _ld(aux) if aux is not None else 0,
-         rowscale, rows_per_scale, residual, _ld(residual) if residual is not None else 0, splitk,
-         out_gelu, _ld(out_gelu) if out_gelu is not None else 0, xsum, c_zstride, xsum_zstride)
+    args = (dt(x.dtype), x, _ld(x), int(x_trans), x_op, w, _ld(w), int(w_trans), w_op, out, _ld(out), out_f32,
+            int(accumulate), M, N, K, float(alpha), bias, act, float(slope), aux, _ld(aux) if aux is not None else 0,
+            rowscale, rows_per_scale, residual, _ld(residual) if residual is not None else 0, splitk,
+            out_gelu, _ld(out_gelu) if out_gelu is not None else 0, xsum, c_zstride, xsum_zstride)
+    if gather is None:
+        call('fw_gemm', *args)
+    else:
+        call('fw_gemm_conv4', *args, *gather, 2 if (x_trans and w_trans) else 1)
     return out
 
 
@@ -320,8 +324,8 @@
                 slot[1].record()
 
 
-def wgrad(g, x, n, k, m, dw, db=None, defer=False):
-    if defer and _in_backward() and _groupable(g, x, n, k, m, dw, db):
+def wgrad(g, x, n, k, m, dw, db=None, defer=False, gather=None):
+    if gather is None and defer and _in_backward() and _groupable(g, x, n, k, m, dw, db):
         _register_flush()
         _pending_w.append((g, x, n, k, m, dw, db))
         return
@@ -329,14 +333,15 @@
     _note_write(db)
     sk = pick_splitk(n, k, m, g.dtype)
     if sk == 1:
-        gemm(g, x, n, k, m, x_trans=True, w_trans=True, out=dw, accumulate=True, xsum=db)
+        gemm(g, x, n, k, m, x_trans=True, w_trans=True, out=dw, accumulate=True, xsum=db, gather=gather)
         return
     nk = (n * k + 3) // 4 * 4
     S = nk + (n + 3) // 4 * 4
     slab = torch.empty((sk, S), dtype=torch.float32, device=g.device)
     cview = slab[0, :n * k].view(n, k)
     xs = slab[0, nk:] if db is not None else None
-    gemm(g, x, n, k, m, x_trans=True, w_trans=True, out=cview, splitk=sk, xsum=xs, c_zstride=S, xsum_zstride=S if db is not None else 0)
+    gemm(g, x, n, k, m, x_trans=True, w_trans=True, out=cview, splitk=sk, xsum=xs, c_zstride=S, xsum_zstride=S if db is not None else 0,
+         gather=gather)
     slab_reduce(slab, sk, n * k, S, dw, db, nk, n, defer=defer)
 
 
@@ -459,6 +464,21 @@
     return col
 
 
+_CONV4_GATHER = int(_os.environ.get('FW_CONV4_GATHER', '1'))
+
+
+def conv4_gather_ok(B, H, W, C, dtype):
+    return bool(_CONV4_GATHER and dtype == torch.bfloat16 and H % 2 == 0 and W % 2 == 0 and C % 4 == 0 and C >= 20
+                and (B * (H // 2) * (W // 2)) % 64 == 0 and (H + 2) * (W + 2) * C < (1 << 30))
+
+
+def pad_cast4(x, B, H, W):
+    C = x.shape[1]
+    xpad = torch.empty((B * (H + 2) * (W + 2), C), dtype=torch.bfloat16, device=x.device)
+    call('fw_pad_cast4', x, _ld(x), xpad, B, H, W, C)
+    return xpad
+
+
 def col2im4(dcol, B, H, W, C, dres=None):
     dx = torch.empty((B * H * W, C), dtype=torch.float32, device=dcol.device)
     call('fw_col2im4', dt(dcol.dtype), dcol, dx, _ld(dx), dres, _ld(dres) if dres is not None else 0, B, H, W, C)
diff --git a/include/fwair.h b/include/fwair.h
--- a/include/fwair.h
+++ b/include/fwair.h
@@ -51,6 +51,14 @@
 int fw_im2col4(int dtype, const float* x, long ldx, void* col, int B, int H, int W, int C, void* stream);
 int fw_col2im4(int dtype, const void* dcol, float* dx, long lddx, const float* dres, long ldr, int B, int H, int W, int C,
                void* stream);
+int fw_pad_cast4(const float* x, long ldx, void* xpad, int B, int H, int W, int C, void* stream);
+int fw_gemm_conv4(int dtype, const void* X, long ldx, int x_trans, int x_op, const void* W, long ldw, int w_trans, int w_op,
+                  void* C, long ldc, int out_f32, int accumulate, int M, int N, int K, float alpha, const float* bias, int act,
+                  float slope, const void* aux, long ldaux, const float* rowscale, int rows_per_scale, const float* residual,
+                  long ldr, int splitk, void* C2, long ldc2, float* xsum, long c_zstride, long xsum_zstride, int B, int H, int W_,
+                  int C_, int gather, void* stream);
+int fw_conv4_offsets(int B, int H, int W, int C, long t0, int n, long* row_off);
+int fw_conv4_k_offsets(int B, int H, int W, int C, int k0, int n, long* k_off);
 int fw_pixel_shuffle(int dtype, const void* g, const float* bias, float* out, long ldo, int B, int H, int W, int Cout,
                      void* stream);
 int fw_pixel_unshuffle(int dtype, const float* dout, long ldo, void* dg, int B, int H, int W, int Cout, void* stream);
```

Result: no change. 344.4 images/sec (median of 6 runs) (+0.8%).
